# Happy-ZZX/PL-VIWO

Measured on AMD Instinct MI355X. Metric: frames/sec (track+EKF update), 752x480 mono, 250 pts+80 lines; ATE vs CPU ref, higher is better.
Workload: dtype f64

## Files before the change

### pl-viwo_amd/csrc/dense_kernels.hip

```cpp
#include "mfma_tile.hpp"
#include "update_kernels.hpp"
#include "wave_ops.hpp"

namespace plv {


static inline int cdiv(int a, int b) { return (a + b - 1) / b; }

__global__ void __launch_bounds__(256) gram_direct_kernel(const double *__restrict__ A, int lda, int nc, const int *__restrict__ acc_rows, int F,
                                                          int mp_max, double *__restrict__ G, const int *__restrict__ skip,
                                                          double *__restrict__ Gs, double *__restrict__ gv) {
  if (skip && *skip == 0) return;
  __shared__ double part[3][256];
  const int nt = (nc + 15) >> 4;
  int rem = blockIdx.x, ti = 0;
  while (rem >= nt - ti) {
    rem -= nt - ti;
    ++ti;
  }
  const int tj = ti + rem;
  const int wave = threadIdx.x >> 6, lane = threadIdx.x & 63, li = lane & 15;
  const double *ai = A + (size_t)min(ti * 16 + li, nc - 1) * lda;
  const double *aj = A + (size_t)min(tj * 16 + li, nc - 1) * lda;
  d4 acc = {0, 0, 0, 0};
  int turn = 0;
  for (int f0 = 0; f0 < F; f0 += 64) {
    const int fr = f0 + lane < F ? acc_rows[f0 + lane] : 0;
    unsigned long long mask = __ballot(fr > 0);
    while (mask) {
      const int b = __ffsll((long long)mask) - 1;
      mask &= mask - 1;
      if ((turn++ & 3) != wave) continue;
      const int rows = min(__shfl(fr, b, 64), mp_max);
      const double *af = ai + (size_t)(f0 + b) * mp_max, *bf = aj + (size_t)(f0 + b) * mp_max;
      auto fa = [&](int, int kk) { return af[kk]; };
      auto fb = [&](int kk, int) { return bf[kk]; };
      acc = mfma_tile_f64_pipe<8>(fa, fb, rows, acc);
    }
  }
  if (wave > 0) {
#pragma unroll
    for (int q = 0; q < 4; ++q) part[wave - 1][q * 64 + lane] = acc[q];
  }
  __syncthreads();
  if (wave == 0) {
#pragma unroll
    for (int q = 0; q < 4; ++q) {
      const double v = ((acc[q] + part[0][q * 64 + lane]) + part[1][q * 64 + lane]) + part[2][q * 64 + lane];
      const int i = ti * 16 + (lane >> 4) + 4 * q, j = tj * 16 + li;
      if (Gs) {
        const int k = nc - 1;
        if (i < k && j < k) Gs[(size_t)j * k + i] = v, Gs[(size_t)i * k + j] = v;
        if (i < k && j == k) gv[i] = v;
      } else if (i < nc && j < nc) {
        G[(size_t)j * nc + i] = v;
      }
    }
  }
}

__global__ void __launch_bounds__(256) ekf_dc_kernel(const double *__restrict__ W, int ldw, int r, int n,
                                                     double *__restrict__ dC, int ldc, double *__restrict__ dx,
                                                     const double *__restrict__ P, int ldp, int *__restrict__ flag, const int *__restrict__ skip,
                                                     const double *__restrict__ dW, const double *__restrict__ C1,
                                                     const double *__restrict__ d0, const int *__restrict__ use_m) {
  if (skip && *skip == 0) return;
  const bool fm = use_m && (use_m[0] | use_m[1]) != 0;
  if (fm) dW = C1;
  const int tn = (n + 1 + 15) >> 4;
  const int ntri = tn * (tn + 1) / 2;
  const int wid = blockIdx.x * 4 + (threadIdx.x >> 6);
  const int lane = threadIdx.x & 63;
  if (wid >= ntri) return;
  int ti = 0, rem = wid;
  while (rem >= tn - ti) {
    rem -= tn - ti;
    ++ti;
  }
  const int tj = ti + rem;
  const double *Wi = W + (size_t)min(ti * 16 + (lane & 15), n) * ldw;
  const double *Wj = W + (size_t)min(tj * 16 + (lane & 15), n) * ldw;
  d4 acc = {0, 0, 0, 0};
  auto fa = [&](int, int kk) { return Wi[kk]; };
  auto fb = [&](int kk, int) { return Wj[kk]; };
  acc = mfma_tile_f64_pipe<16>(fa, fb, r, acc);
#pragma unroll
  for (int q = 0; q < 4; ++q) {
    const int i = ti * 16 + (lane >> 4) + 4 * q, j = tj * 16 + (lane & 15);
    const double v = (dW && i < n && j < n) ? dW[(size_t)j * ldc + i] - acc[q] : acc[q];
    if (i < n && j < n) dC[(size_t)j * ldc + i] = v;
    if (dx && i < n && j == n) dx[i] = fm ? d0[i] - acc[q] : acc[q];
    if (P && i == j && i < n && P[(size_t)i * ldp + i] - v < 0.0) atomicOr(flag, 1);
  }
}

__global__ void __launch_bounds__(256) ekf_commit_kernel(double *__restrict__ P, int ldp, int n,
                                                         const double *__restrict__ dC, int ldc, int *__restrict__ flag,
                                                         const unsigned *__restrict__ mirror_src, unsigned *__restrict__ mirror_dst,
                                                         int mirror_words, const int *__restrict__ skip, double *__restrict__ dx,
                                                         const unsigned *__restrict__ mirror2_src, unsigned *__restrict__ mirror2_dst,
                                                         int mirror2_words,
                                                         int *__restrict__ applied_out, const int *__restrict__ cap_words, int cap,
                                                         double *__restrict__ save, unsigned *__restrict__ save_word, unsigned save_seq) {
  const bool skipped = skip && *skip == 0;
  const bool capped = cap_words && cap_words[0] != 0 && cap_words[1] >= cap;
  if (capped && blockIdx.x == 0) {
    if (threadIdx.x == 0) atomicOr(flag, 16);
    __syncthreads();
  }
  if (applied_out && blockIdx.x == 0 && threadIdx.x == 0) *applied_out = (skipped || capped || *flag != 0) ? 0 : 1;
  if (save_word && blockIdx.x == 0 && threadIdx.x == 0) *save_word = (skipped || capped || *flag != 0) ? 0u : save_seq;
  if (blockIdx.x == 0) {
    if (skipped && dx) {
      for (int i = threadIdx.x; i < n; i += blockDim.x) dx[i] = 0.0;
      __syncthreads();
    }
    if (mirror_dst)
      for (int i = threadIdx.x; i < mirror_words; i += blockDim.x) mirror_dst[i] = mirror_src[i];
  }
  if (mirror2_dst && blockIdx.x == gridDim.x - 1)
    for (int i = threadIdx.x; i < mirror2_words; i += blockDim.x) mirror2_dst[i] = mirror2_src[i];
  if (!(skipped || capped || *flag != 0)) {
    for (int idx = blockIdx.x * blockDim.x + threadIdx.x; idx < n * n; idx += gridDim.x * blockDim.x) {
      int j = idx / n, i = idx - j * n;
      if (i <= j) {
        const double u = P[(size_t)j * ldp + i];
        if (save) save[(size_t)j * n + i] = u, save[(size_t)i * n + j] = P[(size_t)i * ldp + j];
        double v = u - dC[(size_t)j * ldc + i];
        P[(size_t)j * ldp + i] = v;
        P[(size_t)i * ldp + j] = v;
      }
    }
  }
}

bool ekf_fast_fits(int r) { return r <= 192; }
static int launch_ekf_commit(plv_ctx *ctx, double *d_P, int n, int ldp, const double *dC, double *d_dx, int *d_flag, const void *mirror_src,
                             void *mirror_dst, size_t mirror_bytes);

int launch_ekf_fast(plv_ctx *ctx, double *d_P, int n, int ldp, const double *d_H, int r, int k, int ldh, const int *d_cols,
                    const double *d_res, const double *d_Rdiag, double *d_dx, int *d_flag, bool gathered, const void *mirror_src,
                    void *mirror_dst, size_t mirror_bytes) {
  int rc;
  const int ldm = r, ldw = r;
  if ((rc = ctx->d_Mt.reserve((size_t)r * (n + 1 + k) * 8)) || (rc = ctx->d_S.reserve((size_t)r * r * 8 * 2)) ||
      (rc = ctx->d_W.reserve((size_t)r * (n + 1) * 8)) || (rc = ctx->d_y.reserve((size_t)n * n * 8)))
    return rc;
  double *Mt = ctx->d_Mt.as<double>(), *S = ctx->d_S.as<double>(), *W = ctx->d_W.as<double>(), *dC = ctx->d_y.as<double>();
  launch_ekf_ms(ctx, d_P, n, ldp, d_H, r, k, ldh, d_cols, d_Rdiag, Mt, ldm, S, gathered, d_flag);
  if ((rc = launch_bchol_ekf(ctx, S, r, r, Mt, ldm, n, d_res, W, ldw, d_flag))) return rc;
  {
    ProfScope ps(ctx->prof, "ekf_dc_kernel", ctx->stream);
    int tn = cdiv(n + 1, 16);
    int waves = tn * (tn + 1) / 2;
    hipLaunchKernelGGL(ekf_dc_kernel, dim3(cdiv(waves, 4)), dim3(256), 0, ctx->stream, W, ldw, r, n, dC, n, d_dx, d_P, ldp, d_flag, ctx->skip_word,
                       (const double *)nullptr, (const double *)nullptr, (const double *)nullptr, (const int *)nullptr);
  }
  return launch_ekf_commit(ctx, d_P, n, ldp, dC, d_dx, d_flag, mirror_src, mirror_dst, mirror_bytes);
}

static int launch_ekf_commit(plv_ctx *ctx, double *d_P, int n, int ldp, const double *dC, double *d_dx, int *d_flag, const void *mirror_src,
                             void *mirror_dst, size_t mirror_bytes) {
  {
    ProfScope ps(ctx->prof, "ekf_commit_kernel", ctx->stream);
    hipLaunchKernelGGL(ekf_commit_kernel, dim3(std::min(64, cdiv(n * n, 256))), dim3(256), 0, ctx->stream, d_P, ldp, n, dC, n,
                       d_flag, (const unsigned *)mirror_src, (unsigned *)mirror_dst, (int)(mirror_bytes / 4), ctx->skip_word, d_dx,
                       (const unsigned *)(mirror_dst ? ctx->mirror2_src : nullptr), (unsigned *)(mirror_dst ? ctx->mirror2_dst : nullptr),
                       (int)((ctx->mirror2_bytes + 3) / 4), mirror_dst ? ctx->applied_word : nullptr,
                       mirror_dst ? ctx->cap_words : nullptr, ctx->cap, ctx->cov_save, ctx->cov_save_word, ctx->cov_save_seq);
    if (mirror_dst && ctx->applied_word) ctx->applied_used = true;
    if (mirror_dst && ctx->mirror2_dst) ctx->mirror2_taken = true;
  }
  PLV_HIP_CHECK(hipGetLastError());
  return PLV_OK;
}

__global__ void __launch_bounds__(256) cov_restore_kernel(double *__restrict__ P, const double *__restrict__ save, int nn,
                                                          const unsigned *__restrict__ save_word, unsigned seq) {
  if (*save_word != seq) return;
  for (int idx = blockIdx.x * blockDim.x + threadIdx.x; idx < nn; idx += gridDim.x * blockDim.x) P[idx] = save[idx];
}
int launch_cov_restore(plv_ctx *ctx, double *d_P, int n, const double *save, const unsigned *save_word, unsigned seq) {
  hipLaunchKernelGGL(cov_restore_kernel, dim3(std::min(64, cdiv(n * n, 256))), dim3(256), 0, ctx->stream, d_P, save, n * n, save_word, seq);
  PLV_HIP_CHECK(hipGetLastError());
  return PLV_OK;
}

__global__ void __launch_bounds__(256) stack_zero_rejected_kernel(double *__restrict__ A, int lda, int nc, const int *__restrict__ acc_rows, int F, int mp_max) {
  const int f = blockIdx.x;
  if (f >= F) return;
  const int keep = max(acc_rows[f], 0);
  for (int idx = threadIdx.x; idx < nc * mp_max; idx += blockDim.x) {
    const int j = idx / mp_max, i = idx - j * mp_max;
    if (i >= keep) A[(size_t)j * lda + (size_t)f * mp_max + i] = 0.0;
  }
}
__global__ void __launch_bounds__(256) stack_compact_kernel(const double *__restrict__ A, int lda, int nc, const int *__restrict__ acc_rows, int F, int mp_max,
                                                            double *__restrict__ dst, int ldd, int *__restrict__ total_out) {
  __shared__ int s_off;
  const int f = blockIdx.x;
  if (total_out && f == 0 && threadIdx.x < 64) {
    int tot = 0;
    for (int g = threadIdx.x; g < F; g += 64) tot += max(acc_rows[g], 0);
#pragma unroll
    for (int o = 32; o >= 1; o >>= 1) tot += __shfl_xor(tot, o);
    if (threadIdx.x == 0) *total_out = tot;
  }
  const int rows = max(acc_rows[f], 0);
  if (rows == 0) return;
  if (threadIdx.x < 64) {
    int part = 0;
    for (int g = threadIdx.x; g < f; g += 64) part += max(acc_rows[g], 0);
#pragma unroll
    for (int o = 32; o >= 1; o >>= 1) part += __shfl_xor(part, o);
    if (threadIdx.x == 0) s_off = part;
  }
  __syncthreads();
  const int off = s_off;
  if (off + rows > ldd) return;
  for (int idx = threadIdx.x; idx < nc * rows; idx += blockDim.x) {
    const int j = idx / rows, i = idx - j * rows;
    dst[(size_t)j * ldd + off + i] = A[(size_t)j * lda + (size_t)f * mp_max + i];
  }
}
int launch_stack_compact(plv_ctx *ctx, const double *d_A, int lda, int nc, const int *d_acc_rows, int F, int mp_max, double *d_dst, int ldd, bool exact_rows,
                         int *d_total_out) {
  if (!exact_rows) PLV_HIP_CHECK(hipMemsetAsync(d_dst, 0, (size_t)ldd * nc * 8, ctx->stream));
  ProfScope ps(ctx->prof, "stack_compact_kernel", ctx->stream);
  hipLaunchKernelGGL(stack_compact_kernel, dim3(F), dim3(256), 0, ctx->stream, d_A, lda, nc, d_acc_rows, F, mp_max, d_dst, ldd, d_total_out);
  PLV_HIP_CHECK(hipGetLastError());
  return PLV_OK;
}

int launch_stack_zero_rejected(plv_ctx *ctx, double *d_A, int lda, int nc, const int *d_acc_rows, int F, int mp_max) {
  ProfScope ps(ctx->prof, "stack_zero_rejected_kernel", ctx->stream);
  hipLaunchKernelGGL(stack_zero_rejected_kernel, dim3(F), dim3(256), 0, ctx->stream, d_A, lda, nc, d_acc_rows, F, mp_max);
  PLV_HIP_CHECK(hipGetLastError());
  return PLV_OK;
}

__global__ void __launch_bounds__(64) prior_exact_cols_kernel(const double *__restrict__ Lt, int ldl, int k, const int *__restrict__ cols,
                                                              double *__restrict__ W0, int ldw, int *__restrict__ n_near) {
  const int j = blockIdx.x;
  double *dst = W0 + (size_t)cols[j] * ldw;
  const double *src = Lt + (size_t)j * ldl;
  for (int c = threadIdx.x; c < k; c += 64) dst[c] = c <= j ? src[c] : 0.0;
  if (j == 0 && threadIdx.x == 0) {
    n_near[4] = n_near[0];
    n_near[0] = 0;
  }
}

int launch_prior_factor(plv_ctx *ctx, hipStream_t st, const double *d_P, int n, int ldp, const int *d_cols, int k) {
  int rc;
  if ((rc = ctx->d_Lt.reserve((size_t)k * k * 8)) || (rc = ctx->d_W0.reserve((size_t)k * (n + 1) * 8)) ||
      (rc = ctx->d_dW.reserve((size_t)n * n * 8)) || (rc = ctx->d_prior_near.reserve(64)))
    return rc;
  if ((rc = launch_bchol_prior(ctx, st, d_P, ldp, n, d_cols, k, ctx->d_Lt.as<double>(), k, ctx->d_W0.as<double>(), k, ctx->d_prior_near.as<int>()))) return rc;
  {
    ProfScope ps(ctx->prof, "prior_exact_cols_kernel", st);
    hipLaunchKernelGGL(prior_exact_cols_kernel, dim3(k), dim3(64), 0, st, ctx->d_Lt.as<double>(), k, k, d_cols, ctx->d_W0.as<double>(), k,
                       ctx->d_prior_near.as<int>());
  }
  {
    ProfScope ps(ctx->prof, "prior_gain_kernel", st);
    const int tn = cdiv(n + 1, 16), waves = tn * (tn + 1) / 2;
    hipLaunchKernelGGL(ekf_dc_kernel, dim3(cdiv(waves, 4)), dim3(256), 0, st, ctx->d_W0.as<double>(), k, k, n, ctx->d_dW.as<double>(), n,
                       (double *)nullptr, (const double *)nullptr, 0, (int *)nullptr, (const int *)nullptr, (const double *)nullptr,
                       (const double *)nullptr, (const double *)nullptr, (const int *)nullptr);
  }
  PLV_HIP_CHECK(hipGetLastError());
  return PLV_OK;
}

int launch_gram_information(plv_ctx *ctx, const double *d_A, int lda, int nc, const int *d_acc_rows, int F, int mp_max) {
  const int k = nc - 1, nt = cdiv(nc, 16), ntri = nt * (nt + 1) / 2;
  int rc;
  if ((rc = ctx->d_Gs.reserve(((size_t)k * k + k) * 8))) return rc;
  ProfScope ps(ctx->prof, "gram_direct_kernel", ctx->stream);
  hipLaunchKernelGGL(gram_direct_kernel, dim3(ntri), dim3(256), 0, ctx->stream, d_A, lda, nc, d_acc_rows, F, mp_max, (double *)nullptr,
                     ctx->skip_word, ctx->d_Gs.as<double>(), ctx->d_Gs.as<double>() + (size_t)k * k);
  PLV_HIP_CHECK(hipGetLastError());
  return PLV_OK;
}

int launch_ekf_whitened(plv_ctx *ctx, double *d_P, int n, int ldp, int k, const int *d_cols, double *d_dx, int *d_flag, const void *mirror_src,
                        void *mirror_dst, size_t mirror_bytes) {
  int rc;
  if ((rc = ctx->d_Mt.reserve((size_t)k * 8)) || (rc = ctx->d_S.reserve((size_t)k * k * 8)) || (rc = ctx->d_W.reserve((size_t)k * (n + 1) * 8)) ||
      (rc = ctx->d_y.reserve((size_t)n * n * 8)))
    return rc;
  double *cv = ctx->d_Mt.as<double>(), *B = ctx->d_S.as<double>(), *V = ctx->d_W.as<double>(), *dC = ctx->d_y.as<double>();
  const double *Gs = ctx->d_Gs.as<double>(), *gv = Gs + (size_t)k * k;
  if ((rc = ctx->d_C1.reserve(((size_t)n * n + n) * 8)) || (rc = ctx->d_Y0.reserve((size_t)k * (n + 1) * 8)) || (rc = ctx->d_GP.reserve((size_t)k * n * 8)))
    return rc;
  double *Y0 = ctx->d_Y0.as<double>(), *C1 = ctx->d_C1.as<double>(), *d0 = C1 + (size_t)n * n, *GP = ctx->d_GP.as<double>();
  const int *use_m = ctx->d_prior_near.as<int>();
  if (plv::knob(plv::PLV_KNOB_FORCE_FACTOR_FORM)) {
    static const int one[2] = {1, 0};
    PLV_HIP_CHECK(hipMemcpyAsync(ctx->d_prior_near.p, one, 8, hipMemcpyHostToDevice, ctx->stream));
  }
  launch_whiten_b(ctx, ctx->d_Lt.as<double>(), k, Gs, gv, cv, B, d_flag, d_P, ldp, n, d_cols, Y0, GP, d0, use_m);
// ... 13 lines not shown
```

### pl-viwo_amd/csrc/gate_core.hpp

```cpp
#pragma once
#include "blocked_chol.hpp"
#include "gate_stage.hpp"
#include "mfma_tile.hpp"
#include "wave_ops.hpp"

#ifndef GATE_STAMP
#define GATE_STAMP(id)
#endif

namespace plv {

struct GateLds {
  double S[GATE_MMAX * (GATE_MMAX + 1)];
  BcLdsT<2> bc;
  double ybuf[64];
  double passflag;
};

__device__ __forceinline__ double gate_wave_sum(double v) {
#pragma unroll
  for (int off = 32; off > 0; off >>= 1) v += __shfl_xor(v, off, 64);
  return v;
}

struct GateOps {
  static constexpr bool kStoreL = false;
  const double *S;
  const double *r;
  int rstr, mp;
  double *y;
  __device__ __forceinline__ double sym_raw(int i, int c) const {
    const int hi = min(max(i, c), mp - 1), lo = min(min(i, c), mp - 1);
    return S[lo * (GATE_MMAX + 1) + hi];
  }
  __device__ __forceinline__ double border_raw(int, int c) const { return r[(size_t)min(c, mp - 1) * rstr]; }
  __device__ __forceinline__ void scales_ready() const {}
  __device__ __forceinline__ double sym_fix(int i, int c, double g) const { return (i >= mp || c >= mp) ? (i == c ? 1.0 : 0.0) : g; }
  __device__ __forceinline__ double border_fix(int b, int c, double g) const { return (b == 0 && c < mp) ? g : 0.0; }
  __device__ __forceinline__ void store_sym(int, int, double) const {}
  __device__ __forceinline__ void store_border(int b, int c, double v) const {
    if (b == 0 && c < mp) y[c] = v;
  }
};

__host__ __device__ inline int gate_ps_doubles(int k) { return k * (k + 1) / 2 + (k + 1) / 2 + 2; }
__device__ __forceinline__ int gate_tri(int a, int b) {
  const int hi = max(a, b), lo = min(a, b);
  return hi * (hi + 1) / 2 + lo;
}
__device__ __forceinline__ void gate_stage_prior(const GateStage &g, double *Ps, const int *cols_g, int k, int tid, int nthreads) {
  int *cols_l = reinterpret_cast<int *>(Ps + k * (k + 1) / 2);
  for (int i = tid; i < k; i += nthreads) cols_l[i] = cols_g[i];
  const int w = tid >> 6, nw = nthreads >> 6, lane = tid & 63;
  for (int h0 = w; h0 < k; h0 += 8 * nw) {
    double v[8][2];
#pragma unroll
    for (int u = 0; u < 8; ++u) {
      const int hi = min(h0 + u * nw, k - 1);
      const double *row = g.P + (size_t)cols_g[hi] * g.ldp;
#pragma unroll
      for (int c = 0; c < 2; ++c) v[u][c] = row[cols_g[min(lane + 64 * c, hi)]];
    }
#pragma unroll
    for (int u = 0; u < 8; ++u) {
      const int hi = h0 + u * nw;
#pragma unroll
      for (int c = 0; c < 2; ++c) {
        const int lo = lane + 64 * c;
        if (hi < k && lo <= hi) Ps[hi * (hi + 1) / 2 + lo] = v[u][c];
      }
    }
  }
}

__device__ __forceinline__ void gate_tail(const GateStage &g, GateLds &L, const double *Ps, double *T, int f, const double *X, int ncol, int fdim,
                                          int shift, int rows, int k, const int *cols_g) {
  const int wave = threadIdx.x >> 6, lane = threadIdx.x & 63, li = lane & 15, lq = lane >> 4;
  const int mp = rows - fdim;
  const bool valid = shift == fdim && mp >= 1 && mp <= GATE_MMAX && rows >= g.min_rows;
  if (f == 0 && threadIdx.x == 0 && g.n_acc_next) *g.n_acc_next = 0;
  double chi = NAN, nrm2 = 0.0;
  if (valid) {
    const double *Hp = X + (size_t)shift * ncol + fdim;
    if (threadIdx.x == 0) {
      L.bc.bad = 0;
      L.bc.step_flag = 0;
      L.bc.rs_flag = 0;
      L.bc.n_amb = 0;
    }
    const int mt = (mp + 15) >> 4, kt = (k + 15) >> 4;
    const int ngroups = (k + 15) >> 4;
    for (int tj = wave; tj < kt; tj += 4) {
      const int jb = min(tj * 16 + li, k - 1);
      double bv[GATE_KMAX / 4];
#pragma unroll
      for (int u = 0; u < GATE_KMAX / 4; ++u) {
        const int kk = 4 * u + lq;
        const double x = Ps[kk < k ? gate_tri(kk, jb) : 0];
        bv[u] = kk < k ? x : 0.0;
      }
      for (int ti = 0; ti < mt; ++ti) {
        const double *Hr = Hp + (size_t)min(ti * 16 + li, mp - 1) * ncol + lq;
        d4 acc = {0, 0, 0, 0};
#pragma unroll
        for (int gq = 0; gq < GATE_KMAX / 16; ++gq)
          if (gq < ngroups) {
            double av[4];
#pragma unroll
            for (int u = 0; u < 4; ++u) av[u] = (16 * gq + 4 * u + lq < k) ? Hr[16 * gq + 4 * u] : 0.0;
#pragma unroll
            for (int u = 0; u < 4; ++u) acc = __builtin_amdgcn_mfma_f64_16x16x4f64(av[u], bv[4 * gq + u], acc, 0, 0, 0);
          }
#pragma unroll
        for (int q = 0; q < 4; ++q) {
          const int i = ti * 16 + lq + 4 * q, j = tj * 16 + li;
          if (i < mp && j < k) T[i * GATE_TLD + j] = acc[q];
        }
      }
    }
    __syncthreads();
    GATE_STAMP(6);
    for (int t = wave; t < mt * mt; t += 4) {
      const int ti = t / mt, tj = t - ti * mt;
      if (tj < ti) continue;
      const double *Tr = T + (size_t)min(ti * 16 + li, mp - 1) * GATE_TLD;
      const double *Hr = Hp + (size_t)min(tj * 16 + li, mp - 1) * ncol;
      d4 acc = {0, 0, 0, 0};
      auto fa = [&](int, int kk) { return Tr[kk]; };
      auto fb = [&](int kk, int) { return Hr[kk]; };
      acc = mfma_tile_f64_pipe<16>(fa, fb, k, acc);
#pragma unroll
      for (int q = 0; q < 4; ++q) {
        const int i = ti * 16 + lq + 4 * q, j = tj * 16 + li;
        if (i < mp && j < mp) L.S[i * (GATE_MMAX + 1) + j] = acc[q] + (i == j ? g.sigma2 : 0.0);
      }
    }
    __syncthreads();
    GATE_STAMP(7);
    if (wave == 0) {
      const double rv = lane < mp ? Hp[(size_t)lane * ncol + k] : 0.0;
      nrm2 = gate_wave_sum(rv * rv);
    }
    GateOps ops{L.S, Hp + k, ncol, mp, L.ybuf};
    blocked_chol<2>(ops, L.bc, mp, 1, 0.0, 0);
    __syncthreads();
    GATE_STAMP(8);
    if (wave == 0) {
      const double y = lane < mp ? L.ybuf[lane] : 0.0;
      chi = gate_wave_sum(y * y);
      if (L.bc.bad) chi = NAN;
    }
  }
  if (wave == 0 && lane == 0) {
    g.chi2[f] = chi;
    if (g.dec) g.dec[3 * f] = valid ? chi : NAN, g.dec[3 * f + 1] = (valid && mp < g.q95_n) ? g.chi2_mult * g.q95[mp] : NAN, g.dec[3 * f + 2] = valid ? sqrt(nrm2) : NAN;
    bool pass = valid && !isnan(chi);
    if (pass && g.res_norm_gate > 0.0) pass = sqrt(nrm2) < g.res_norm_gate;
    if (pass) pass = (mp < g.q95_n) && (chi < g.chi2_mult * g.q95[mp]);
    g.accepted[f] = pass ? 1 : 0;
    const bool overflow = shift == fdim && mp > GATE_MMAX;
    if (g.acc_rows) g.acc_rows[f] = pass ? mp : (overflow ? -1 : 0);
    if (g.h_accepted) g.h_accepted[f] = pass ? 1 : 0;
    if (g.h_acc_rows) g.h_acc_rows[f] = pass ? mp : (overflow ? -1 : 0);
    if (pass && g.n_acc) atomicAdd(g.n_acc, 1);
    L.passflag = pass ? 1.0 : 0.0;
  }
  if (g.probe_dst) {
    for (int i = threadIdx.x; i < g.probe_stride_a; i += blockDim.x) g.probe_dst[(size_t)f * g.probe_stride_a + i] = g.probe_src[(size_t)f * g.probe_stride_a + i];
    for (int i = threadIdx.x; i < g.probe_stride_b; i += blockDim.x)
      g.probe_dst[(size_t)g.probe_off_b + (size_t)f * g.probe_stride_b + i] = g.probe_src[(size_t)g.probe_off_b + (size_t)f * g.probe_stride_b + i];
  }
  if (g.stack) {
    __syncthreads();
    const bool pass = L.passflag != 0.0;
    if (!pass && g.stack_accepted_only) return;
    const double *Hp = X + (size_t)shift * ncol + fdim;
    double *dst = g.stack + (size_t)f * g.mp_max;
    const int rows_w = g.stack_accepted_only ? mp : g.mp_max;
    for (int i = threadIdx.x & 31; i < rows_w; i += 32)
      for (int j = threadIdx.x >> 5; j <= k; j += 8) {
        double v = 0.0;
        if (pass && i < mp) v = Hp[(size_t)i * ncol + j];
        dst[(size_t)j * g.lds + i] = v;
      }
  }
}

}
```

### pl-viwo_amd/csrc/jacobian_kernels.hip

```cpp
#include <hip/hip_runtime.h>
namespace plv {
#define JAC_NSTAMP 32
__device__ long long *g_jac_stamps = nullptr;
__device__ __forceinline__ void jac_stamp(int id) {
  long long *s = g_jac_stamps;
  if (s && threadIdx.x == 0) s[blockIdx.x * JAC_NSTAMP + id] = (long long)__builtin_amdgcn_s_memtime();
}
}
#define GATE_STAMP(id) jac_stamp(id)
#include "cam_models.hpp"
#include "gate_core.hpp"
#include "jacobian_kernels.hpp"
#include "nullspace_core.hpp"

namespace plv {

struct V3 {
  double v[3];
  __device__ double &operator[](int i) { return v[i]; }
  __device__ double operator[](int i) const { return v[i]; }
};
struct M3 {
  double m[9];
  __device__ double &operator()(int r, int c) { return m[3 * r + c]; }
// ... 615 lines not shown
  for (int i = 0; i < 2; ++i)
#pragma unroll
    for (int j = 0; j < 3; ++j) {
      hx[(size_t)(P.col_ext + j) * cstr + (2 * c + i) * rstr] = wz[3 * i] * sk(0, j) + wz[3 * i + 1] * sk(1, j) + wz[3 * i + 2] * sk(2, j);
      hx[(size_t)(P.col_ext + 3 + j) * cstr + (2 * c + i) * rstr] = wz[3 * i + j];
    }
}
__device__ __forceinline__ void rows_write_int(const JacParams &P, int c, const double *Wm, const double *dzeta, double *hx, int cstr, int rstr) {
  if (P.col_int < 0) return;
#pragma unroll
  for (int j = 0; j < 8; ++j) {
    hx[(size_t)(P.col_int + j) * cstr + (2 * c) * rstr] = Wm[0] * dzeta[j] + Wm[1] * dzeta[8 + j];
    hx[(size_t)(P.col_int + j) * cstr + (2 * c + 1) * rstr] = Wm[2] * dzeta[j] + Wm[3] * dzeta[8 + j];
  }
}

__device__ void jacobian_rows_core(const JacParams &P, int f, int o, int s0, double tm, int c, const Interp &jac, M3 R_GtoI, V3 p_IinG, double *hf,
                                   double *hx, double *rs, int cstr, int rstr) {
  double r2[2], dzn[4], dzeta[16], dznp[6], dpC_dI[18], Wm[4], wz[6], WI[12];
  M3 dpC_dpG;
  V3 lever;
  const V3 pf = ldV(P.p_FinG + 3 * f), pf_fej = ldV(P.p_FinG_fej + 3 * f);
  rows_est_part(P, pf, P.obs_uv + 2 * o, R_GtoI, p_IinG, r2, dzn, dzeta);
  rows_fej_part(P, pf_fej, jac.R, jac.p, dznp, dpC_dpG, dpC_dI, lever);
  rows_whiten_part(P, o, rows_at_clone(P, tm), dzn, dznp, dpC_dI, Wm, wz, WI);
  rows_write_res(c, Wm, r2, rs, rstr);
  rows_write_hf(P, pf_fej, c, wz, dpC_dpG, hf, cstr, rstr);
#pragma unroll
  for (int w = 0; w < 4; ++w) rows_write_pose(P.clone_col[s0 + w], c, WI, jac.Ho[w], jac.lam[w], hx, cstr, rstr);
  rows_write_dt(P, c, WI, jac.dtj, hx, cstr, rstr);
  rows_write_ext(P, c, wz, lever, hx, cstr, rstr);
  rows_write_int(P, c, Wm, dzeta, hx, cstr, rstr);
}

__device__ __forceinline__ void tri_wave_sync() {
  __builtin_amdgcn_fence(__ATOMIC_RELEASE, "workgroup");
  __builtin_amdgcn_wave_barrier();
  __builtin_amdgcn_fence(__ATOMIC_ACQUIRE, "workgroup");
}
#define PRE_STRIDE 127
#define LPRE_STRIDE 113
enum { LPRE_R2 = 70, LPRE_DZLI = 72, LPRE_ATC = 84, LPRE_WM = 85, LPRE_WLI = 89, LPRE_WI = 101 };
enum { PRE_R = 0, PRE_P = 9, PRE_HO = 12, PRE_LAM = 48, PRE_DTJ = 52, PRE_RE = 58, PRE_PE = 67,
       PRE_R2 = 70, PRE_DZN = 72, PRE_DZETA = 76, PRE_ATC = 92, PRE_WM = 93, PRE_WZ = 97, PRE_WI = 103, PRE_G = 115, PRE_LEVER = 124 };
__device__ __forceinline__ void pre_store_jac(double *pre, const Interp &j) {
#pragma unroll
  for (int i = 0; i < 9; ++i) pre[PRE_R + i] = j.R.m[i];
#pragma unroll
  for (int i = 0; i < 3; ++i) pre[PRE_P + i] = j.p[i];
#pragma unroll
  for (int w = 0; w < 4; ++w) {
#pragma unroll
    for (int i = 0; i < 9; ++i) pre[PRE_HO + 9 * w + i] = j.Ho[w].m[i];
    pre[PRE_LAM + w] = j.lam[w];
  }
#pragma unroll
  for (int i = 0; i < 6; ++i) pre[PRE_DTJ + i] = j.dtj[i];
}
__device__ __forceinline__ void pre_load_jac(const double *pre, Interp &j) {
#pragma unroll
  for (int i = 0; i < 9; ++i) j.R.m[i] = pre[PRE_R + i];
#pragma unroll
  for (int i = 0; i < 3; ++i) j.p[i] = pre[PRE_P + i];
#pragma unroll
  for (int w = 0; w < 4; ++w) {
#pragma unroll
    for (int i = 0; i < 9; ++i) j.Ho[w].m[i] = pre[PRE_HO + 9 * w + i];
    j.lam[w] = pre[PRE_LAM + w];
  }
#pragma unroll
  for (int i = 0; i < 6; ++i) j.dtj[i] = pre[PRE_DTJ + i];
}
__device__ __forceinline__ int assign_row_slots(const JacParams &P, int o0, int o1, int ld, const double *tm_l , int *s0_l, int *slot_l) {
  const int lane = threadIdx.x & 63;
  int base = 0;
  for (int ob = o0; ob < o1; ob += 64) {
    const int o = ob + lane;
    const bool have = o < o1;
    const double tm = (have ? tm_l[o - o0] : 0.0) + P.cam_dt;
    const int s0 = have ? bounding_start(P, tm) : -1;
    const unsigned long long vmask = __ballot(s0 >= 0);
    const int c = base + __popcll(vmask & ((1ull << lane) - 1ull));
    base += __popcll(vmask);
    if (have) {
      s0_l[o - o0] = s0;
      slot_l[o - o0] = (s0 >= 0 && 2 * c + 2 <= ld) ? c : -1;
    }
  }
  return base;
}
__device__ __forceinline__ void est_pose_tab(const JacParams &P, const WinTab &T, int o, int s0, double tm, M3 &R_GtoI, V3 &p_IinG) {
  if (P.res_R) {
    R_GtoI = ldM(P.res_R + 9 * o);
    p_IinG = ldV(P.res_p + 3 * o);
  } else {
    Interp est;
    interpolate_tab(P, T, s0, tm, false, est);
    R_GtoI = est.R;
    p_IinG = est.p;
  }
}

__device__ __forceinline__ void jacobian_rows_split(const JacParams &P, const V3 &pf, const V3 &pf_fej, int o0, int n_o, const int *s0_l,
                                                    const int *slot_l, const double *tm_l, const float *uv_l, double *pre, double *X, int ncol, int k) {
  const int wave = threadIdx.x >> 6, lane = threadIdx.x & 63;
  double *hf = X, *hx = X + 3, *rs = X + 3 + k;
  for (int ib = 0; ib < n_o; ib += 64) {
    const int i = ib + lane;
    const int c = i < n_o ? slot_l[i] : -1;
    const int o = o0 + i;
    double *pr = pre + (size_t)max(c, 0) * PRE_STRIDE;
    double dznp[6], dpC_dI[18];
    if (c >= 0) {
      if (wave == 0) {
        M3 dpC_dpG;
        V3 lever;
        rows_fej_part(P, pf_fej, ldM(pr + PRE_R), ldV(pr + PRE_P), dznp, dpC_dpG, dpC_dI, lever);
#pragma unroll
        for (int q = 0; q < 9; ++q) pr[PRE_G + q] = dpC_dpG.m[q];
#pragma unroll
        for (int q = 0; q < 3; ++q) pr[PRE_LEVER + q] = lever[q];
      } else if (wave == 1 && P.cam_model == PLV_CAM_EQUIDISTANT) {
        rows_est_part(P, pf, uv_l + 2 * i, ldM(pr + PRE_RE), ldV(pr + PRE_PE), pr + PRE_R2, pr + PRE_DZN, pr + PRE_DZETA);
      } else if (wave == 1) {
        double r2[2], dzn[4], dzeta[16];
        rows_est_part(P, pf, uv_l + 2 * i, ldM(pr + PRE_RE), ldV(pr + PRE_PE), r2, dzn, dzeta);
        pr[PRE_R2] = r2[0], pr[PRE_R2 + 1] = r2[1];
#pragma unroll
        for (int q = 0; q < 4; ++q) pr[PRE_DZN + q] = dzn[q];
#pragma unroll
        for (int q = 0; q < 16; ++q) pr[PRE_DZETA + q] = dzeta[q];
      } else if (wave == 2) {
        pr[PRE_ATC] = rows_at_clone(P, tm_l[i] + P.cam_dt) ? 1.0 : 0.0;
      }
    }
    __syncthreads();
    if (c >= 0 && wave == 0) {
      double dzn[4], Wm[4], wz[6], WI[12];
#pragma unroll
      for (int q = 0; q < 4; ++q) dzn[q] = pr[PRE_DZN + q];
      rows_whiten_part(P, o, pr[PRE_ATC] != 0.0, dzn, dznp, dpC_dI, Wm, wz, WI);
#pragma unroll
      for (int q = 0; q < 4; ++q) pr[PRE_WM + q] = Wm[q];
#pragma unroll
      for (int q = 0; q < 6; ++q) pr[PRE_WZ + q] = wz[q];
#pragma unroll
      for (int q = 0; q < 12; ++q) pr[PRE_WI + q] = WI[q];
    }
    __syncthreads();
    if (c >= 0) {
      double WI[12];
#pragma unroll
      for (int q = 0; q < 12; ++q) WI[q] = pr[PRE_WI + q];
      rows_write_pose(P.clone_col[s0_l[i] + wave], c, WI, ldM(pr + PRE_HO + 9 * wave), pr[PRE_LAM + wave], hx, 1, ncol);
      if (wave == 0) {
        double Wm[4], r2[2] = {pr[PRE_R2], pr[PRE_R2 + 1]}, dtj[6];
#pragma unroll
        for (int q = 0; q < 4; ++q) Wm[q] = pr[PRE_WM + q];
#pragma unroll
        for (int q = 0; q < 6; ++q) dtj[q] = pr[PRE_DTJ + q];
        rows_write_res(c, Wm, r2, rs, ncol);
        rows_write_dt(P, c, WI, dtj, hx, 1, ncol);
      } else if (wave == 1) {
        double wz[6];
#pragma unroll
        for (int q = 0; q < 6; ++q) wz[q] = pr[PRE_WZ + q];
        rows_write_ext(P, c, wz, ldV(pr + PRE_LEVER), hx, 1, ncol);
      } else if (wave == 2) {
        double Wm[4], dzeta[16];
#pragma unroll
        for (int q = 0; q < 4; ++q) Wm[q] = pr[PRE_WM + q];
#pragma unroll
        for (int q = 0; q < 16; ++q) dzeta[q] = pr[PRE_DZETA + q];
        rows_write_int(P, c, Wm, dzeta, hx, 1, ncol);
      } else {
        double wz[6];
#pragma unroll
        for (int q = 0; q < 6; ++q) wz[q] = pr[PRE_WZ + q];
        rows_write_hf(P, pf_fej, c, wz, ldM(pr + PRE_G), hf, 1, ncol);
      }
    }
    __syncthreads();
  }
}

struct FusedLds {
  int ns, tab, tri, pre, cam, idx, end;
};
__host__ __device__ inline FusedLds fused_lds_layout(int ld, int ncol, int fdim, int n_tab, int max_obs, bool with_tri) {
  const bool lines = fdim == 6;
  FusedLds L;
  L.ns = ld * ncol;
  L.tab = (L.ns + nullspace_wy_scratch(ld, fdim) + 7) & ~7;
  L.tri = L.tab + n_tab * (int)(sizeof(WinTab) / 8);
  L.pre = L.tri + (with_tri && !lines ? tri_smem_doubles(max_obs) : 0);
  L.cam = L.pre + (ld / 2 < max_obs ? ld / 2 : max_obs) * (lines ? LPRE_STRIDE : PRE_STRIDE);
  L.idx = L.cam + max_obs * 12 * (lines ? 2 : 1);
  L.end = L.idx + (lines ? 5 : 3) * max_obs + (max_obs * (lines ? 13 : 9) + 7) / 8 + 1;
  return L;
}
static_assert(sizeof(WinTab) % 8 == 0, "fused_lds_layout counts WinTab in doubles");

__global__ void __launch_bounds__(256) __attribute__((amdgpu_waves_per_eu(2))) jacobian_nullspace_kernel(JacParams P, int F, GatherArgs g, PointTriStage tri, GateStage gate) {
  extern __shared__ double jsm[];
  __shared__ int s_rows, s_base;
  __shared__ double tri_tot[32], s_tri[5];
  __shared__ double s_ct[JAC_MAX_WIN / 2 + 3];
  __shared__ int s_ccol[JAC_MAX_WIN / 2 + 3];
  if ((int)blockIdx.x >= F) {
    gather_cov_block(g, blockIdx.x - F);
    return;
  }
  int f = blockIdx.x;
  if (P.spec_order) {
    if ((int)blockIdx.x >= *P.spec_count) return;
    f = P.spec_order[blockIdx.x];
  }
  const int wave = threadIdx.x >> 6, lane = threadIdx.x & 63;
  double touch = 0.0;
  for (int off = threadIdx.x * 128; off < P.in_bytes; off += 256 * 128) touch += *(const volatile double *)(P.in_base + off);
  const int ld = P.ld, k = P.k, ncol = 3 + k + 1, max_obs = tri.max_obs;
  const FusedLds lay = fused_lds_layout(ld, ncol, 3, 2 * max(P.n_clones - 3, 0), max_obs, tri.on != 0);
  double *X = jsm, *piv = jsm + lay.ns, *tri_smem = jsm + lay.tri, *pre = jsm + lay.pre, *cam = jsm + lay.cam;
  WinTab *tab = reinterpret_cast<WinTab *>(jsm + lay.tab);
  double *tm_l = jsm + lay.idx;
  float *uv_l = reinterpret_cast<float *>(tm_l + max_obs), *uvn_l = uv_l + 2 * max_obs;
  int *s0_l = reinterpret_cast<int *>(uvn_l + 2 * max_obs), *slot_l = s0_l + max_obs;
  unsigned char *valid_l = reinterpret_cast<unsigned char *>(slot_l + max_obs);
  jac_stamp(0);
  const int o0 = P.obs_ptr[f], o1 = P.obs_end ? P.obs_end[f] : P.obs_ptr[f + 1];
  if ((int)threadIdx.x < P.n_clones) s_ct[threadIdx.x] = P.clone_time[threadIdx.x], s_ccol[threadIdx.x] = P.clone_col[threadIdx.x];
  for (int i = threadIdx.x; i < o1 - o0; i += blockDim.x) {
    tm_l[i] = P.obs_time[o0 + i];
    uv_l[2 * i] = P.obs_uv[2 * (o0 + i)], uv_l[2 * i + 1] = P.obs_uv[2 * (o0 + i) + 1];
    if (tri.on) uvn_l[2 * i] = tri.uvn[2 * (o0 + i)], uvn_l[2 * i + 1] = tri.uvn[2 * (o0 + i) + 1];
  }
  for (int i = threadIdx.x; i < ld * ncol; i += blockDim.x) X[i] = 0.0;
  if (f == 0 && P.cols_out)
    for (int i = threadIdx.x; i < k; i += blockDim.x) P.cols_out[i] = P.cols_in[i];
  __syncthreads();
  P.clone_time = s_ct, P.clone_col = s_ccol;
  if (wave == 0) {
    const int base = assign_row_slots(P, o0, o1, ld, tm_l, s0_l, slot_l);
    if (lane == 0) s_base = base;
    jac_stamp(15);
  }
  build_window_tables(P, tab);
  jac_stamp(2);
  if (wave == 0) {
    for (int i = lane; i < o1 - o0; i += 64) {
      const int s0 = s0_l[i], c = slot_l[i];
      valid_l[i] = s0 >= 0;
      if (s0 < 0) continue;
      M3 R_GtoI;
      V3 p_IinG;
      est_pose_tab(P, tab[2 * s0], o0 + i, s0, tm_l[i] + P.cam_dt, R_GtoI, p_IinG);
      if (c >= 0) {
        double *pr = pre + (size_t)c * PRE_STRIDE;
#pragma unroll
        for (int q = 0; q < 9; ++q) pr[PRE_RE + q] = R_GtoI.m[q];
#pragma unroll
        for (int q = 0; q < 3; ++q) pr[PRE_PE + q] = p_IinG[q];
      }
      if (tri.on) {
        const M3 R_GtoC = mm(ldM(P.R_ItoC), R_GtoI);
        const V3 p_CinG = vsub(p_IinG, mv(tp(R_GtoC), ldV(P.p_IinC)));
#pragma unroll
        for (int q = 0; q < 9; ++q) cam[12 * i + q] = R_GtoC.m[q];
#pragma unroll
        for (int q = 0; q < 3; ++q) cam[12 * i + 9 + q] = p_CinG[q];
      }
    }
    if (tri.on) {
      tri_wave_sync();
      triangulate_feature(P, f, 0, o1 - o0, cam, valid_l, uvn_l, uv_l, tri.opt, tri.p_out, tri.ok_out, tri.err_out, max_obs, tri_smem, tri_tot, true, s_tri);
    }
  } else {
    for (int i = threadIdx.x - 64; i < o1 - o0; i += 192) {
      const int c = slot_l[i];
      if (c < 0) continue;
      Interp jac;
      const int s0 = s0_l[i];
      interpolate_tab(P, tab[2 * s0 + 1], s0, tm_l[i] + P.cam_dt, true, jac);
      pre_store_jac(pre + (size_t)c * PRE_STRIDE, jac);
    }
    if (gate.on) gate_stage_prior(gate, reinterpret_cast<double *>(reinterpret_cast<char *>(jsm) + gate.ps_off), P.cols_in, k, threadIdx.x - 64, 192);
  }
  __threadfence_block();
  __syncthreads();
  jac_stamp(1);
  bool selected;
  V3 pf, pf_fej;
  if (tri.on) {
    selected = P.sel_flags[f] && s_tri[3] != 0.0 && s_tri[4] < 3.0;
    pf = pf_fej = ldV(s_tri);
  } else {
    selected = !P.tri_ok || candidate_selected(P, f);
    pf = ldV(P.p_FinG + 3 * f), pf_fej = ldV(P.p_FinG_fej + 3 * f);
  }
  if (selected) {
    jacobian_rows_split(P, pf, pf_fej, o0, o1 - o0, s0_l, slot_l, tm_l, uv_l, pre, X, ncol, k);
    if (threadIdx.x == 0) {
      s_rows = min(2 * s_base, ld & ~1);
      P.rows[f] = 2 * s_base;
      if (P.spec_pass) atomicAdd(P.spec_pass, 1);
    }
  } else if (threadIdx.x == 0) {
    s_rows = 0;
    P.rows[f] = 0;
  }
  __syncthreads();
  jac_stamp(3);
  const int rows = s_rows;
  GateLds &gl = *reinterpret_cast<GateLds *>(reinterpret_cast<char *>(jsm) + gate.lds_off);
  const double *gPs = reinterpret_cast<const double *>(reinterpret_cast<char *>(jsm) + gate.ps_off);
  double *gT = reinterpret_cast<double *>(reinterpret_cast<char *>(jsm) + gate.t_off);
  if ((tri.on || P.tri_ok) && rows == 0) {
    if (gate.on) gate_tail(gate, gl, gPs, gT, f, X, ncol, 3, 0, 0, k, P.cols_in);
    return;
  }
  const int shift = rows > 3 ? 3 : 0;
  if (shift) nullspace_householder_wy<3>(X, piv, rows, ncol);
  jac_stamp(4);
  double *hf = P.Hf + (size_t)f * 3 * ld, *hx = P.Hx + (size_t)f * k * ld, *rs = P.res + (size_t)f * ld;
  for (int j = gate.on ? ncol : (int)threadIdx.x; j < ncol; j += blockDim.x) {
    double *dst = j < 3 ? hf + j * ld : (j < 3 + k ? hx + (size_t)(j - 3) * ld : rs);
    const int off = j < 3 ? 0 : shift;
    for (int i0 = 0; i0 < ld; i0 += 8) {
      double v[8];
#pragma unroll
      for (int u = 0; u < 8; ++u) {
        const int r = i0 + u + off;
        v[u] = r < ld ? X[r * ncol + j] : 0.0;
      }
#pragma unroll
      for (int u = 0; u < 8; ++u)
        if (i0 + u < ld) dst[i0 + u] = v[u];
    }
  }
  jac_stamp(5);
  if (gate.on) gate_tail(gate, gl, gPs, gT, f, X, ncol, 3, shift, min(rows, ld), k, P.cols_in);
  if (touch == 1.2345678e300) P.rows[f] = -1;
  jac_stamp(9);
}

__device__ __forceinline__ void campose_one(const JacParams &P, int o, double *__restrict__ poses , unsigned char *__restrict__ valid,
                            double *__restrict__ imu) {
  const double tm = P.obs_time[o] + P.cam_dt;
  const int s0 = bounding_start(P, tm);
  valid[o] = s0 >= 0;
  if (s0 < 0) return;
  M3 R_GtoI;
  V3 p_IinG;
  if (P.res_R) {
    R_GtoI = ldM(P.res_R + 9 * o);
    p_IinG = ldV(P.res_p + 3 * o);
  } else {
    Interp est;
    interpolate(P, s0, tm, false, false, est);
    R_GtoI = est.R;
    p_IinG = est.p;
  }
  if (imu) {
#pragma unroll
    for (int i = 0; i < 9; ++i) imu[12 * o + i] = R_GtoI.m[i];
#pragma unroll
    for (int i = 0; i < 3; ++i) imu[12 * o + 9 + i] = p_IinG[i];
  }
  const M3 R_GtoC = mm(ldM(P.R_ItoC), R_GtoI);
  const V3 p_CinG = vsub(p_IinG, mv(tp(R_GtoC), ldV(P.p_IinC)));
#pragma unroll
  for (int i = 0; i < 9; ++i) poses[12 * o + i] = R_GtoC.m[i];
#pragma unroll
  for (int i = 0; i < 3; ++i) poses[12 * o + 9 + i] = p_CinG[i];
}

__device__ int cpi_find(const double *t, int n, double x) {
  int lo = 0, hi = n;
  while (lo < hi) {
    const int mid = (lo + hi) >> 1;
    if (t[mid] < x) lo = mid + 1; else hi = mid;
  }
  return (lo < n && t[lo] == x) ? lo : -1;
}
__device__ int clone_find(const CpiParams &C, double x) {
  for (int i = 0; i < C.n_clones; ++i)
    if (C.clone_time[i] == x) return i;
  return -1;
}
__global__ void __launch_bounds__(64) cpi_pose_kernel(CpiParams C, const double *__restrict__ tq, double *__restrict__ Rout,
                                                      double *__restrict__ pout, unsigned char *__restrict__ ok) {
  const int q = blockIdx.x * blockDim.x + threadIdx.x;
  if (q >= C.n_q) return;
  ok[q] = 0;
  const double t = tq[q];
  const int n = C.n;
  M3 R_I0toIk;
  V3 alpha;
  double clone_t, dt;
  const int e = cpi_find(C.t, n, t);
  if (e >= 0 && clone_find(C, C.clone_t[e]) >= 0) {
    R_I0toIk = ldM(C.R + 9 * e);
    alpha = ldV(C.alpha + 3 * e);
    clone_t = C.clone_t[e];
    dt = C.dt[e];
  } else {
    if (n == 0 || t < C.t[0] || t > C.t[n - 1]) return;
    int lo = 0, hi = n;
    while (lo < hi) {
      const int mid = (lo + hi) >> 1;
      if (C.t[mid] < t) lo = mid + 1; else hi = mid;
    }
    const int i0 = (t == C.t[0]) ? 0 : lo - 1;
    int up = lo;
    while (up < n && C.t[up] <= t) ++up;
    const int i1 = (t == C.t[n - 1]) ? n - 1 : up;
    if (C.clone_t[i0] != C.clone_t[i1]) return;
    if (C.clone_t[i0] < C.clone_time[0]) return;
    const double lambda = (t - C.t[i0]) / (C.t[i1] - C.t[i0]);
    const M3 R0 = ldM(C.R + 9 * i0), R1 = ldM(C.R + 9 * i1);
    R_I0toIk = mm(exp_so3(vsc(log_so3(mm(R1, tp(R0))), lambda)), R0);
    const V3 a0 = ldV(C.alpha + 3 * i0), a1 = ldV(C.alpha + 3 * i1);
    alpha = vadd(vsc(a0, 1 - lambda), vsc(a1, lambda));
    clone_t = C.clone_t[i0];
    dt = t - clone_t;
  }
  const int ci = clone_find(C, clone_t), vi = cpi_find(C.t, n, clone_t);
  if (ci < 0 || vi < 0) return;
  const M3 RGtoI0 = ldM(C.clone_R + 9 * ci);
  const V3 p0 = ldV(C.clone_p + 3 * ci), v0 = ldV(C.v + 3 * vi);
  const V3 g{{C.gravity[0], C.gravity[1], C.gravity[2]}};
  const M3 RGtoI = mm(R_I0toIk, RGtoI0);
  V3 p = vadd(p0, vsc(v0, dt));
  p = vsub(p, vsc(vsc(vsc(g, 0.5), dt), dt));
  p = vadd(p, mv(tp(RGtoI0), alpha));
#pragma unroll
  for (int i = 0; i < 9; ++i) Rout[9 * q + i] = RGtoI.m[i];
#pragma unroll
  for (int i = 0; i < 3; ++i) pout[3 * q + i] = p[i];
// ... 412 lines not shown
#pragma unroll
    for (int j = 0; j < 3; ++j) {
      double so = 0, sp = 0;
#pragma unroll
      for (int q = 0; q < 3; ++q) {
        so += a[6 * i + q] * A00(q, j);
        sp += a[6 * i + q] * A03(q, j);
      }
#pragma unroll
      for (int q = 0; q < 3; ++q) {
        so += a[6 * i + 3 + q] * A30(q, j);
        sp += a[6 * i + 3 + q] * 0.0;
      }
      x[6 * i + j] = so;
      x[6 * i + 3 + j] = sp;
    }
}
__device__ __forceinline__ void line_whiten_part(const JacParams &P, int o, bool at_clone, const double *dzli, const M3 &A00, const M3 &A30, const M3 &A03,
                                                 double *Wm, double *wli, double *WI) {
  double HI[12];
  line_times_dli(dzli, A00, A30, A03, HI);
  double Rn[4] = {P.sigma_pix * P.sigma_pix, 0, 0, P.sigma_pix * P.sigma_pix};
  if (!at_clone && P.use_pol_cov) {
#pragma unroll
    for (int i = 0; i < 2; ++i)
#pragma unroll
      for (int j = 0; j < 2; ++j) {
        double s = 0;
#pragma unroll
        for (int q = 0; q < 6; ++q) s += HI[6 * i + q] * (q < 3 ? P.intr_ori_cov : P.intr_pos_cov) * HI[6 * j + q];
        Rn[2 * i + j] += s;
      }
  } else if (!at_clone && P.use_imu_cov) {
    add_imu_cov(P, o, HI, Rn);
  }
  const double l00 = sqrt(Rn[0]), l10 = Rn[2] / l00, l11 = sqrt(Rn[3] - l10 * l10);
  const double m00 = sqrt(l00), m10 = l10 / m00, m11 = sqrt(l11 - m10 * m10);
#pragma unroll
  for (int col = 0; col < 2; ++col) {
    const double b0 = col == 0 ? 1.0 : 0.0, b1 = col == 1 ? 1.0 : 0.0;
    const double y0 = b0 / m00, y1 = (b1 - m10 * y0) / m11;
    const double x1 = y1 / m11, x0 = (y0 - m10 * x1) / m00;
    Wm[col] = x0;
    Wm[2 + col] = x1;
  }
#pragma unroll
  for (int j = 0; j < 6; ++j) {
    wli[j] = Wm[0] * dzli[j] + Wm[1] * dzli[6 + j];
    wli[6 + j] = Wm[2] * dzli[j] + Wm[3] * dzli[6 + j];
  }
  line_times_dli(wli, A00, A30, A03, WI);
}
__device__ __forceinline__ void line_write_hf(int c, const double *wli, const M3 &Re, const M3 &Rsk, double *hf, int cstr, int rstr) {
#pragma unroll
  for (int i = 0; i < 2; ++i)
#pragma unroll
    for (int j = 0; j < 3; ++j) {
      double a = 0, b = 0;
#pragma unroll
      for (int q = 0; q < 3; ++q) {
        a += wli[6 * i + q] * Re(q, j);
        b += wli[6 * i + q] * Rsk(q, j);
      }
#pragma unroll
      for (int q = 0; q < 3; ++q) {
        a += wli[6 * i + 3 + q] * 0.0;
        b += wli[6 * i + 3 + q] * Re(q, j);
      }
      hf[(size_t)j * cstr + (2 * c + i) * rstr] = a;
      hf[(size_t)(3 + j) * cstr + (2 * c + i) * rstr] = b;
    }
}

__device__ void line_rows(const JacParams &P, int l, int o, int s0, double tm, int c, double *hf, double *hx, double *rs, int cstr,
                          int rstr, const WinTab *tab = nullptr) {
  const V3 nG = ldV(P.line_FinG + 6 * l), vG = ldV(P.line_FinG + 6 * l + 3);
  Interp jac;
  if (tab)
    interpolate_tab(P, tab[2 * s0 + 1], s0, tm, true, jac);
  else
    interpolate(P, s0, tm, true, true, jac);
  M3 Re;
  V3 pe;
  if (P.res_R) {
    Re = ldM(P.res_R + 9 * o);
    pe = ldV(P.res_p + 3 * o);
  } else {
    Interp est;
    if (tab)
      interpolate_tab(P, tab[2 * s0], s0, tm, false, est);
    else
      interpolate(P, s0, tm, false, false, est);
    Re = est.R;
    pe = est.p;
  }
  double r2[2], dzli[12], Wm[4], wli[12], WI[12];
  M3 Rsk, A00, A30, A03;
  line_est_part(P, nG, vG, P.seg_uv + 4 * o, Re, pe, r2, dzli, Rsk);
  line_fej_part(nG, vG, jac.R, jac.p, A00, A30, A03);
  line_whiten_part(P, o, rows_at_clone(P, tm), dzli, A00, A30, A03, Wm, wli, WI);
  rows_write_res(c, Wm, r2, rs, rstr);
  line_write_hf(c, wli, Re, Rsk, hf, cstr, rstr);
#pragma unroll
  for (int w = 0; w < 4; ++w) rows_write_pose(P.clone_col[s0 + w], c, WI, jac.Ho[w], jac.lam[w], hx, cstr, rstr);
  rows_write_dt(P, c, WI, jac.dtj, hx, cstr, rstr);
}

__global__ void __launch_bounds__(64) line_jacobian_kernel(JacParams P) {
  const int l = blockIdx.x;
  const int ld = P.ld, k = P.k;
  double *hf = P.Hf + (size_t)l * 6 * ld, *hx = P.Hx + (size_t)l * k * ld, *rs = P.res + (size_t)l * ld;
  for (int i = threadIdx.x; i < 6 * ld; i += 64) hf[i] = 0.0;
  for (int i = threadIdx.x; i < k * ld; i += 64) hx[i] = 0.0;
  for (int i = threadIdx.x; i < ld; i += 64) rs[i] = 0.0;
  __syncthreads();
  if (P.tri_ok && !candidate_selected(P, l)) {
    if (threadIdx.x == 0) P.rows[l] = 0;
    return;
  }
  const int o0 = P.obs_ptr[l], o1 = P.obs_ptr[l + 1];
  int base = 0;
  for (int ob = o0; ob < o1; ob += 64) {
    const int o = ob + threadIdx.x;
    const bool have = o < o1;
    const double tm = (have ? P.obs_time[o] : 0.0) + P.cam_dt;
    const int s0 = have ? bounding_start(P, tm) : -1;
    const unsigned long long vmask = __ballot(s0 >= 0);
    const int c = base + __popcll(vmask & ((1ull << threadIdx.x) - 1ull));
    base += __popcll(vmask);
    if (s0 >= 0 && 2 * c + 2 <= ld) line_rows(P, l, o, s0, tm, c, hf, hx, rs, ld, 1);
  }
  if (threadIdx.x == 0) P.rows[l] = 2 * base;
}

__device__ void line_triangulate_one(const JacParams &P, int l, int o0, int o1, const double *cam, const double *imu, const unsigned char *valid,
                                     const float *seg_uvn, const double *anchor, bool has_anchor, double *out, unsigned char &ok);
struct LineTriStage {
  int on, max_obs;
  double *cam, *imu;
  unsigned char *valid;
  double *out_g;
  unsigned char *ok_g;
};
__device__ __forceinline__ void line_rows_split(const JacParams &P, const V3 &nG, const V3 &vG, int o0, int n_o, const int *s0_l, const int *slot_l,
                                                const double *tm_l, const float *seg_l, double *pre, double *X, int ncol, int k) {
  const int wave = threadIdx.x >> 6, lane = threadIdx.x & 63;
  double *hf = X, *hx = X + 6, *rs = X + 6 + k;
  for (int ib = 0; ib < n_o; ib += 64) {
    const int i = ib + lane;
    const int c = i < n_o ? slot_l[i] : -1;
    const int o = o0 + i;
    double *pr = pre + (size_t)max(c, 0) * LPRE_STRIDE;
    M3 A00, A30, A03;
    M3 Re, Rsk;
    if (c >= 0) {
      if (wave == 0) {
        line_fej_part(nG, vG, ldM(pr + PRE_R), ldV(pr + PRE_P), A00, A30, A03);
      } else if (wave == 1) {
        double r2[2], dzli[12];
        Re = ldM(pr + PRE_RE);
        line_est_part(P, nG, vG, seg_l + 4 * i, Re, ldV(pr + PRE_PE), r2, dzli, Rsk);
        pr[LPRE_R2] = r2[0], pr[LPRE_R2 + 1] = r2[1];
#pragma unroll
        for (int q = 0; q < 12; ++q) pr[LPRE_DZLI + q] = dzli[q];
      } else if (wave == 2) {
        pr[LPRE_ATC] = rows_at_clone(P, tm_l[i] + P.cam_dt) ? 1.0 : 0.0;
      }
    }
    __syncthreads();
    if (c >= 0 && wave == 0) {
      double dzli[12], Wm[4], wli[12], WI[12];
#pragma unroll
      for (int q = 0; q < 12; ++q) dzli[q] = pr[LPRE_DZLI + q];
      line_whiten_part(P, o, pr[LPRE_ATC] != 0.0, dzli, A00, A30, A03, Wm, wli, WI);
#pragma unroll
      for (int q = 0; q < 4; ++q) pr[LPRE_WM + q] = Wm[q];
#pragma unroll
      for (int q = 0; q < 12; ++q) pr[LPRE_WLI + q] = wli[q], pr[LPRE_WI + q] = WI[q];
    }
    __syncthreads();
    if (c >= 0) {
      double WI[12];
#pragma unroll
      for (int q = 0; q < 12; ++q) WI[q] = pr[LPRE_WI + q];
      rows_write_pose(P.clone_col[s0_l[i] + wave], c, WI, ldM(pr + PRE_HO + 9 * wave), pr[PRE_LAM + wave], hx, 1, ncol);
      if (wave == 0) {
        double Wm[4], r2[2] = {pr[LPRE_R2], pr[LPRE_R2 + 1]}, dtj[6];
#pragma unroll
        for (int q = 0; q < 4; ++q) Wm[q] = pr[LPRE_WM + q];
#pragma unroll
        for (int q = 0; q < 6; ++q) dtj[q] = pr[PRE_DTJ + q];
        rows_write_res(c, Wm, r2, rs, ncol);
        rows_write_dt(P, c, WI, dtj, hx, 1, ncol);
      } else if (wave == 1) {
        double wli[12];
#pragma unroll
        for (int q = 0; q < 12; ++q) wli[q] = pr[LPRE_WLI + q];
        line_write_hf(c, wli, Re, Rsk, hf, 1, ncol);
      }
    }
    __syncthreads();
  }
}

__device__ __forceinline__ void jpl_left_update_dev(const double *Qin, const double *d, double *M) {
  double a[3] = {0.5 * d[0], 0.5 * d[1], 0.5 * d[2]}, b = 1.0;
  const double nd = sqrt(a[0] * a[0] + a[1] * a[1] + a[2] * a[2] + 1.0);
  a[0] /= nd, a[1] /= nd, a[2] /= nd, b /= nd;
  const double v[3] = {Qin[0], Qin[1], Qin[2]}, w0 = Qin[3];
  double r[4];
  r[0] = b * v[0] - (a[1] * v[2] - a[2] * v[1]) + a[0] * w0;
  r[1] = b * v[1] - (a[2] * v[0] - a[0] * v[2]) + a[1] * w0;
  r[2] = b * v[2] - (a[0] * v[1] - a[1] * v[0]) + a[2] * w0;
  r[3] = -(a[0] * v[0] + a[1] * v[1] + a[2] * v[2]) + b * w0;
  if (r[3] < 0) {
#pragma unroll
    for (int i = 0; i < 4; ++i) r[i] = -r[i];
  }
  const double nr = sqrt(r[0] * r[0] + r[1] * r[1] + r[2] * r[2] + r[3] * r[3]);
  double Q[4];
#pragma unroll
  for (int i = 0; i < 4; ++i) Q[i] = r[i] / nr;
  const double x = Q[0], y = Q[1], z = Q[2], w = Q[3], c = 2 * w * w - 1;
  M[0] = c + 2 * x * x, M[1] = 2 * w * z + 2 * x * y, M[2] = -2 * w * y + 2 * x * z;
  M[3] = -2 * w * z + 2 * y * x, M[4] = c + 2 * y * y, M[5] = 2 * w * x + 2 * y * z;
  M[6] = 2 * w * y + 2 * z * x, M[7] = -2 * w * x + 2 * z * y, M[8] = c + 2 * z * z;
}

__global__ void __launch_bounds__(256) line_jacobian_nullspace_kernel(JacParams P, int L, GatherArgs g, JacParams Pt, LineTriStage tri, GateStage gate) {
  extern __shared__ double jsm[];
  __shared__ int s_rows, s_base, s_ok;
  __shared__ double s_line[6];
  __shared__ double s_ct[JAC_MAX_WIN / 2 + 3];
  __shared__ int s_ccol[JAC_MAX_WIN / 2 + 3];
  __shared__ double s_cR[(JAC_MAX_WIN / 2 + 3) * 9], s_cp[(JAC_MAX_WIN / 2 + 3) * 3], s_cal[9 + 3 + 8 + 1], s_anchor[3];
  __shared__ unsigned char s_has;
  if (P.chain_dx && *P.chain_status != 0) return;
  if ((int)blockIdx.x >= L) {
    gather_cov_block(g, blockIdx.x - L);
    return;
  }
  const int l = blockIdx.x, wave = threadIdx.x >> 6, lane = threadIdx.x & 63;
  double touch = 0.0;
  for (int off = threadIdx.x * 128; off < P.in_bytes; off += 256 * 128) touch += *(const volatile double *)(P.in_base + off);
  const int ld = P.ld, k = P.k, ncol = 6 + k + 1, max_obs = tri.max_obs, nwin = max(P.n_clones - 3, 0);
  const FusedLds lay = fused_lds_layout(ld, ncol, 6, (tri.on ? 3 : 2) * nwin, max_obs, tri.on != 0);
  double *X = jsm, *piv = jsm + lay.ns, *pre = jsm + lay.pre, *cam = jsm + lay.cam, *imu = cam + (size_t)max_obs * 12;
  WinTab *tab = reinterpret_cast<WinTab *>(jsm + lay.tab);
  double *tm_l = jsm + lay.idx;
  float *uv_l = reinterpret_cast<float *>(tm_l + max_obs), *uvn_l = uv_l + 4 * max_obs;
  int *s0_l = reinterpret_cast<int *>(uvn_l + 4 * max_obs), *slot_l = s0_l + max_obs, *s0t_l = slot_l + max_obs;
  unsigned char *valid_l = reinterpret_cast<unsigned char *>(s0t_l + max_obs);
  jac_stamp(0);
  const int o0 = P.obs_ptr[l], o1 = P.obs_ptr[l + 1];
  if ((int)threadIdx.x < P.n_clones) s_ct[threadIdx.x] = P.clone_time[threadIdx.x], s_ccol[threadIdx.x] = P.clone_col[threadIdx.x];
  for (int i = threadIdx.x; i < o1 - o0; i += blockDim.x) {
    tm_l[i] = P.obs_time[o0 + i];
#pragma unroll
    for (int q = 0; q < 4; ++q) uv_l[4 * i + q] = P.seg_uv[4 * (o0 + i) + q];
    if (tri.on)
#pragma unroll
      for (int q = 0; q < 4; ++q) uvn_l[4 * i + q] = Pt.seg_uvn[4 * (o0 + i) + q];
  }
  for (int i = threadIdx.x; i < ld * ncol; i += blockDim.x) X[i] = 0.0;
  if (l == 0 && P.cols_out)
    for (int i = threadIdx.x; i < k; i += blockDim.x) P.cols_out[i] = P.cols_in[i];
  __syncthreads();
  P.clone_time = s_ct, P.clone_col = s_ccol, Pt.clone_time = s_ct;
  if (P.chain_dx && *P.chain_applied != 0) {
    const double *dx = P.chain_dx;
    const int N = P.n_clones, t = threadIdx.x;
    if (t < N) {
      const int id = P.chain_id[t];
#pragma unroll
      for (int q = 0; q < 3; ++q) s_cp[3 * t + q] = id >= 0 ? P.clone_p[3 * t + q] + dx[id + 3 + q] : P.clone_p[3 * t + q];
      if (id >= 0) {
        jpl_left_update_dev(P.chain_q + 4 * t, dx + id, s_cR + 9 * t);
      } else {
#pragma unroll
        for (int q = 0; q < 9; ++q) s_cR[9 * t + q] = P.clone_R[9 * t + q];
      }
    } else if (t == 64) {
      const int id = P.chain_id[N];
      if (id >= 0) {
        jpl_left_update_dev(P.chain_qe, dx + id, s_cal);
#pragma unroll
        for (int q = 0; q < 3; ++q) s_cal[9 + q] = P.p_IinC[q] + dx[id + 3 + q];
      } else {
#pragma unroll
        for (int q = 0; q < 9; ++q) s_cal[q] = P.R_ItoC[q];
#pragma unroll
        for (int q = 0; q < 3; ++q) s_cal[9 + q] = P.p_IinC[q];
      }
    } else if (t == 65) {
      const int id = P.chain_id[N + 1];
#pragma unroll
      for (int q = 0; q < 8; ++q) s_cal[12 + q] = id >= 0 ? P.K[q] + dx[id + q] : P.K[q];
    } else if (t == 66) {
      const int id = P.chain_id[N + 2];
      s_cal[20] = id >= 0 ? P.cam_dt + dx[id] : P.cam_dt;
    }
    __syncthreads();
    P.clone_R = s_cR, P.clone_p = s_cp;
#pragma unroll
    for (int q = 0; q < 9; ++q) P.R_ItoC[q] = s_cal[q];
#pragma unroll
    for (int q = 0; q < 3; ++q) P.p_IinC[q] = s_cal[9 + q];
#pragma unroll
    for (int q = 0; q < 8; ++q) P.K[q] = s_cal[12 + q];
    P.cam_dt = s_cal[20];
  }
  if (wave == 0) {
    const int base = assign_row_slots(P, o0, o1, ld, tm_l, s0_l, slot_l);
    if (lane == 0) s_base = base;
    jac_stamp(15);
  } else if (wave == 1 && tri.on) {
    for (int i = lane; i < o1 - o0; i += 64) s0t_l[i] = bounding_start(Pt, tm_l[i] + Pt.cam_dt);
  }
  build_window_tables(P, tab, tri.on ? Pt.clone_R : nullptr, tri.on ? Pt.clone_p : nullptr);
  jac_stamp(2);
  if (wave == 0) {
    if (tri.on) {
      for (int i = lane; i < o1 - o0; i += 64) {
        const int s0 = s0t_l[i];
        valid_l[i] = s0 >= 0;
        if (s0 < 0) continue;
        M3 R_GtoI;
        V3 p_IinG;
        est_pose_tab(Pt, tab[2 * nwin + s0], o0 + i, s0, tm_l[i] + Pt.cam_dt, R_GtoI, p_IinG);
#pragma unroll
        for (int q = 0; q < 9; ++q) imu[12 * i + q] = R_GtoI.m[q];
#pragma unroll
        for (int q = 0; q < 3; ++q) imu[12 * i + 9 + q] = p_IinG[q];
        const M3 R_GtoC = mm(ldM(Pt.R_ItoC), R_GtoI);
        const V3 p_CinG = vsub(p_IinG, mv(tp(R_GtoC), ldV(Pt.p_IinC)));
#pragma unroll
        for (int q = 0; q < 9; ++q) cam[12 * i + q] = R_GtoC.m[q];
#pragma unroll
        for (int q = 0; q < 3; ++q) cam[12 * i + 9 + q] = p_CinG[q];
      }
      if (Pt.anc_ptr && lane == 0) {
        unsigned char has = 0;
        for (int c = Pt.anc_ptr[l]; c < Pt.anc_ptr[l + 1] && !has; ++c) {
          const int pf = Pt.anc_f[c];
          if (pf >= 0 && Pt.anc_tri_ok[pf]) {
            s_anchor[0] = Pt.anc_tri_p[3 * pf], s_anchor[1] = Pt.anc_tri_p[3 * pf + 1], s_anchor[2] = Pt.anc_tri_p[3 * pf + 2];
            has = 1;
          } else if (Pt.anc_has_old[c]) {
            s_anchor[0] = Pt.anc_old[3 * c], s_anchor[1] = Pt.anc_old[3 * c + 1], s_anchor[2] = Pt.anc_old[3 * c + 2];
            has = 1;
          }
        }
        s_has = has;
      }
      tri_wave_sync();
      jac_stamp(10);
      double out_l[6] = {0, 0, 0, 0, 0, 0};
      unsigned char ok_l = 0;
      const bool has_anchor = Pt.anc_ptr ? s_has != 0 : (Pt.has_pt && Pt.has_pt[l]);
      line_triangulate_one(Pt, l, 0, o1 - o0, cam, imu, valid_l, uvn_l, Pt.anc_ptr ? s_anchor : Pt.anchor_pt + 3 * l, has_anchor, out_l, ok_l);
      if (lane == 0) {
#pragma unroll
        for (int i = 0; i < 6; ++i) tri.out_g[6 * l + i] = out_l[i], s_line[i] = out_l[i];
        tri.ok_g[l] = ok_l;
        s_ok = ok_l;
      }
    }
  } else {
    for (int i = threadIdx.x - 64; i < o1 - o0; i += 192) {
      const int c = slot_l[i];
      if (c < 0) continue;
      const int s0 = s0_l[i];
      double *pr = pre + (size_t)c * LPRE_STRIDE;
      Interp jac;
      interpolate_tab(P, tab[2 * s0 + 1], s0, tm_l[i] + P.cam_dt, true, jac);
      pre_store_jac(pr, jac);
      M3 Re;
      V3 pe;
      est_pose_tab(P, tab[2 * s0], o0 + i, s0, tm_l[i] + P.cam_dt, Re, pe);
#pragma unroll
      for (int q = 0; q < 9; ++q) pr[PRE_RE + q] = Re.m[q];
#pragma unroll
      for (int q = 0; q < 3; ++q) pr[PRE_PE + q] = pe[q];
    }
    if (gate.on) gate_stage_prior(gate, reinterpret_cast<double *>(reinterpret_cast<char *>(jsm) + gate.ps_off), P.cols_in, k, threadIdx.x - 64, 192);
  }
  __threadfence_block();
  __syncthreads();
  jac_stamp(1);
  bool selected;
  V3 nG, vG;
  if (tri.on) {
    selected = P.sel_flags[l] && s_ok;
    nG = ldV(s_line), vG = ldV(s_line + 3);
  } else {
    selected = !P.tri_ok || candidate_selected(P, l);
    nG = ldV(P.line_FinG + 6 * l), vG = ldV(P.line_FinG + 6 * l + 3);
  }
  if (selected) {
    line_rows_split(P, nG, vG, o0, o1 - o0, s0_l, slot_l, tm_l, uv_l, pre, X, ncol, k);
    if (threadIdx.x == 0) {
      s_rows = min(2 * s_base, ld & ~1);
      P.rows[l] = 2 * s_base;
    }
  } else if (threadIdx.x == 0) {
    s_rows = 0;
    P.rows[l] = 0;
  }
  __syncthreads();
  jac_stamp(3);
  const int rows = s_rows;
  GateLds &gl = *reinterpret_cast<GateLds *>(reinterpret_cast<char *>(jsm) + gate.lds_off);
  const double *gPs = reinterpret_cast<const double *>(reinterpret_cast<char *>(jsm) + gate.ps_off);
  double *gT = reinterpret_cast<double *>(reinterpret_cast<char *>(jsm) + gate.t_off);
  if ((tri.on || P.tri_ok) && rows == 0) {
    if (gate.on) gate_tail(gate, gl, gPs, gT, l, X, ncol, 6, 0, 0, k, P.cols_in);
    return;
  }
  const int shift = rows > 6 ? 6 : 0;
  if (shift) nullspace_householder_wy<6>(X, piv, rows, ncol);
  jac_stamp(4);
  double *hf = P.Hf + (size_t)l * 6 * ld, *hx = P.Hx + (size_t)l * k * ld, *rs = P.res + (size_t)l * ld;
  for (int j = gate.on ? ncol : (int)threadIdx.x; j < ncol; j += blockDim.x) {
    double *dst = j < 6 ? hf + j * ld : (j < 6 + k ? hx + (size_t)(j - 6) * ld : rs);
    const int off = j < 6 ? 0 : shift;
    for (int i0 = 0; i0 < ld; i0 += 8) {
      double v[8];
#pragma unroll
      for (int u = 0; u < 8; ++u) {
        const int r = i0 + u + off;
        v[u] = r < ld ? X[r * ncol + j] : 0.0;
      }
#pragma unroll
      for (int u = 0; u < 8; ++u)
        if (i0 + u < ld) dst[i0 + u] = v[u];
    }
  }
  jac_stamp(5);
  if (gate.on) gate_tail(gate, gl, gPs, gT, l, X, ncol, 6, shift, min(rows, ld), k, P.cols_in);
  if (touch == 1.2345678e300) P.rows[l] = -1;
  jac_stamp(9);
}

__device__ void line_triangulate_one(const JacParams &P, int l, int o0, int o1, const double *cam, const double *imu, const unsigned char *valid,
                                     const float *seg_uvn, const double *anchor, bool has_anchor, double *out, unsigned char &ok);
__global__ void __launch_bounds__(64) line_triangulate_kernel(JacParams P, double *cam, double *imu, unsigned char *valid, double *out_g,
                                                              unsigned char *ok_g) {
  const int l = blockIdx.x;
  const int o0 = P.obs_ptr[l], o1 = P.obs_ptr[l + 1];
  for (int o = o0 + (int)threadIdx.x; o < o1; o += 64) campose_one(P, o, cam, valid, imu);
  __threadfence_block();
  __syncthreads();
  double out_l[6] = {0, 0, 0, 0, 0, 0};
  unsigned char ok_l = 0;
  line_triangulate_one(P, l, o0, o1, cam, imu, valid, P.seg_uvn, P.anchor_pt + 3 * l, P.has_pt && P.has_pt[l], out_l, ok_l);
  if (threadIdx.x == 0) {
#pragma unroll
    for (int i = 0; i < 6; ++i) out_g[6 * l + i] = out_l[i];
    ok_g[l] = ok_l;
  }
}
__device__ void line_triangulate_one(const JacParams &P, int l, int o0, int o1, const double *cam, const double *imu, const unsigned char *valid,
                                     const float *seg_uvn, const double *anchor, bool has_anchor, double *out , unsigned char &ok) {
  int first = -1, nvalid = 0;
  for (int o = o0; o < o1; ++o)
    if (valid[o]) {
      if (first < 0) first = o;
      ++nvalid;
    }
  if (nvalid < 2) return;
  const int D = P.lineD ? P.lineD[l] : 0;
  if (D > 0 && has_anchor) {
    const M3 R = ldM(imu + 12 * first);
    const V3 e{{D == 1 ? 1.0 : 0.0, D == 2 ? 1.0 : 0.0, D == 3 ? 1.0 : 0.0}};
    const V3 dir = mv(tp(R), e);
    const V3 mom = cross3(ldV(anchor), dir);
#pragma unroll
    for (int i = 0; i < 3; ++i) {
      out[i] = mom[i];
      out[3 + i] = dir[i];
    }
    ok = 1;
    return;
  }
  const M3 R0 = ldM(cam + 12 * first);
  const V3 p0 = ldV(cam + 12 * first + 9);
  const float *u0 = seg_uvn + 4 * first;
  const V3 p11{{(double)u0[0], (double)u0[1], 1.0}}, p12{{(double)u0[2], (double)u0[3], 1.0}};
  const V3 n0 = cross3(p11, p12);
  const double pl0[4] = {n0[0], n0[1], n0[2], 0.0};
  V3 dsum{{0, 0, 0}}, nsum{{0, 0, 0}};
  double dnorm = 0;
  int cnt = 0;
  for (int o = first + 1; o < o1; ++o) {
    if (!valid[o]) continue;
    const M3 Ri = ldM(cam + 12 * o);
    const V3 pi = ldV(cam + 12 * o + 9);
    const M3 R0i = mm(Ri, tp(R0));
    const V3 pi0 = mv(R0, vsub(pi, p0));
    const float *um = seg_uvn + 4 * o;
    V3 p31{{(double)um[0], (double)um[1], 1.0}}, p32{{(double)um[2], (double)um[3], 1.0}};
    p31 = vadd(mv(tp(R0i), p31), pi0);
    p32 = vadd(mv(tp(R0i), p32), pi0);
    const V3 nn = cross3(vsub(p31, pi0), vsub(p32, pi0));
    const double pl1[4] = {nn[0], nn[1], nn[2], -dot3(pi0, cross3(p31, p32))};
    V3 n1{{pl0[0], pl0[1], pl0[2]}}, n2{{pl1[0], pl1[1], pl1[2]}};
    n1 = vsc(n1, 1 / vnorm(n1));
    n2 = vsc(n2, 1 / vnorm(n2));
    const double cth = dot3(n1, n2) / (vnorm(n1) * vnorm(n2));
    if (fabs(cth) >= 0.99) continue;
#define PLV_DP(i, j) (pl0[i] * pl1[j] - pl1[i] * pl0[j])
    const V3 head{{PLV_DP(0, 3), PLV_DP(1, 3), PLV_DP(2, 3)}}, tail{{-PLV_DP(1, 2), PLV_DP(0, 2), -PLV_DP(0, 1)}};
#undef PLV_DP
    dsum = vadd(dsum, tail);
    nsum = vadd(nsum, head);
    dnorm += vnorm(tail);
    ++cnt;
  }
  if (cnt == 0) return;
  const V3 rhead = vsc(dsum, 1 / dnorm), rtail = vsc(nsum, 1.0 / cnt);
  const M3 R0t = tp(R0);
  const V3 vW = mv(R0t, rhead);
  const V3 nW = vadd(mv(R0t, rtail), mv(skew3(p0), mv(R0t, rhead)));
#pragma unroll
  for (int i = 0; i < 3; ++i) {
    out[i] = nW[i];
    out[3 + i] = vW[i];
  }
  ok = 1;
}

#define TRY_STAMP(x)          \
  do {                        \
    const int _rc = (x);      \
    if (_rc != PLV_OK) return _rc; \
  } while (0)
struct JacStampHost {
  bool on = plv::knob(plv::PLV_KNOB_KERNEL_STAMPS);
  long long *d = nullptr;
  int cap = 0;
  struct Acc {
    const char *name;
    double sum[JAC_NSTAMP] = {}, mx[JAC_NSTAMP] = {}, slowest = 0;
    long n[JAC_NSTAMP] = {}, launches = 0;
  } acc[2] = {{"tri_jacobian_nullspace_kernel"}, {"line_tri_jacobian_nullspace_kernel"}};
  int arm(hipStream_t s, int blocks) {
    if (blocks > cap) {
      if (d) (void)hipFree(d);
      cap = blocks + 64;
      PLV_HIP_CHECK(hipMalloc(&d, (size_t)cap * JAC_NSTAMP * 8));
      PLV_HIP_CHECK(hipMemcpyToSymbol(HIP_SYMBOL(g_jac_stamps), &d, sizeof(d)));
    }
    PLV_HIP_CHECK(hipMemsetAsync(d, 0, (size_t)blocks * JAC_NSTAMP * 8, s));
    return PLV_OK;
  }
  int collect(hipStream_t s, int blocks, int which) {
    PLV_HIP_CHECK(hipStreamSynchronize(s));
    std::vector<long long> h((size_t)blocks * JAC_NSTAMP);
    PLV_HIP_CHECK(hipMemcpy(h.data(), d, h.size() * 8, hipMemcpyDeviceToHost));
    Acc &a = acc[which];
    double slow = 0;
    for (int b = 0; b < blocks; ++b) {
      const long long *t = &h[(size_t)b * JAC_NSTAMP];
      if (!t[0] || !t[9]) continue;
      slow = std::max(slow, (double)(t[9] - t[0]));
      if (!t[4]) continue;
      for (int i = 1; i < JAC_NSTAMP; ++i)
        if (t[i]) a.sum[i] += (double)(t[i] - t[0]), a.mx[i] = std::max(a.mx[i], (double)(t[i] - t[0])), ++a.n[i];
    }
    a.slowest += slow;
    ++a.launches;
    return PLV_OK;
  }
  ~JacStampHost() {
    if (!on) return;
    static const char *label[JAC_NSTAMP] = {"start", "triangulated", "window tables", "rows built", "null space", "block written", "gate: T", "gate: S",
                                            "gate: factor", "end", "tri: camera poses", "tri: linear solve", "tri: refined", "gate: map staged", "gate: T first column", "row slots",
                                            "LM pass 1", "LM pass 2", "LM pass 3", "LM pass 4", "LM pass 5", "LM pass 6", "LM pass 7", "LM pass 8", "LM pass 9", "LM pass 10", "LM pass 11", "LM pass 12+",
                                            "", "", "", ""};
    static const int order[] = {15, 2, 10, 11, 16, 17, 18, 19, 20, 21, 22, 23, 24, 25, 26, 27, 12, 1, 3, 4, 5, 13, 14, 6, 7, 8, 9};
    for (const Acc &a : acc) {
      if (!a.launches) continue;
      fprintf(stderr, "[plv stamps] %s: %ld launches, slowest workgroup %.0f cycles on average\n", a.name, a.launches, a.slowest / (double)a.launches);
      for (int i : order)
        if (a.n[i]) fprintf(stderr, "[plv stamps]   %-20s @ %8.0f mean  %8.0f max  (%ld workgroups)\n", label[i], a.sum[i] / (double)a.n[i], a.mx[i], a.n[i]);
    }
  }
};
static JacStampHost &jac_stamps() {
  static JacStampHost h;
  return h;
}

int launch_line_jacobians(plv_ctx *ctx, const JacParams &P) {
  ProfScope ps(ctx->prof, "line_jacobian_kernel", ctx->stream);
  hipLaunchKernelGGL(line_jacobian_kernel, dim3(P.n_feat), dim3(64), 0, ctx->stream, P);
  PLV_HIP_CHECK(hipGetLastError());
  return PLV_OK;
}

int launch_line_jacobians_projected(plv_ctx *ctx, const JacParams &P, const GatherArgs *g, int gather_blocks, const JacParams *Pt, double *d_cam,
                                    double *d_imu, unsigned char *d_valid, double *d_lines, unsigned char *d_ok, int max_obs) {
  ProfScope ps(ctx->prof, Pt ? "line_tri_jacobian_nullspace_kernel" : "line_jacobian_nullspace_kernel", ctx->stream);
  if (2 * (P.n_clones - 3) > JAC_MAX_WIN) {
    set_last_error("line jacobians: %d clones exceed the window table (%d)", P.n_clones, JAC_MAX_WIN / 2 + 3);
    return PLV_E_CAPACITY;
  }
  max_obs = std::max(max_obs, 1);
  const FusedLds lay = fused_lds_layout(P.ld, 6 + P.k + 1, 6, (Pt ? 3 : 2) * std::max(P.n_clones - 3, 0), max_obs, Pt != nullptr);
  size_t shm = (size_t)lay.end * sizeof(double);
  const size_t lds_cap = 160 * 1024 - static_smem_bytes((const void *)line_jacobian_nullspace_kernel);
  if (shm > lds_cap) {
    set_last_error("line jacobians: block of %zu bytes exceeds LDS", shm);
    return PLV_E_CAPACITY;
  }
  GatherArgs none{};
  LineTriStage tri{Pt ? 1 : 0, max_obs, d_cam, d_imu, d_valid, d_lines, d_ok};
  GateStage gate = ctx->gate_stage;
  ctx->gate_stage.on = 0;
  const size_t gate_off = ((size_t)lay.tab * sizeof(double) + 63) & ~(size_t)63;
  const size_t t_off = (gate_off + sizeof(GateLds) + 63) & ~(size_t)63;
  const size_t ps_off = (std::max(shm, t_off + (size_t)GATE_MMAX * GATE_TLD * sizeof(double)) + 63) & ~(size_t)63;
  const size_t gate_end = ps_off + (size_t)gate_ps_doubles(P.k) * sizeof(double);
  if (P.k > GATE_KMAX || gate_end > lds_cap) gate.on = 0;
  if (gate.on) {
    gate.lds_off = (int)gate_off, gate.ps_off = (int)ps_off, gate.t_off = (int)t_off;
    shm = gate_end;
  }
  ctx->gate_stage_taken = gate.on != 0;
  PLV_HIP_CHECK(ensure_dyn_smem((const void *)line_jacobian_nullspace_kernel, (int)shm));
  if (jac_stamps().on) TRY_STAMP(jac_stamps().arm(ctx->stream, P.n_feat));
  hipLaunchKernelGGL(line_jacobian_nullspace_kernel, dim3(P.n_feat + (g ? gather_blocks : 0)), dim3(256), shm, ctx->stream, P, P.n_feat,
                     g ? *g : none, Pt ? *Pt : P, tri, gate);
  PLV_HIP_CHECK(hipGetLastError());
  if (jac_stamps().on) TRY_STAMP(jac_stamps().collect(ctx->stream, P.n_feat, 1));
  return PLV_OK;
}

int launch_triangulate_lines(plv_ctx *ctx, const JacParams &P, double *d_poses, double *d_imu, unsigned char *d_valid,
                             double *d_lines, unsigned char *d_ok) {
  {
    ProfScope ps(ctx->prof, "line_triangulate_kernel", ctx->stream);
    hipLaunchKernelGGL(line_triangulate_kernel, dim3(P.n_feat), dim3(64), 0, ctx->stream, P, d_poses, d_imu, d_valid, d_lines, d_ok);
  }
  PLV_HIP_CHECK(hipGetLastError());
  return PLV_OK;
}

int launch_triangulate(plv_ctx *ctx, const JacParams &P, double *d_poses, unsigned char *d_valid, const float *d_uvn,
                       const plv_tri_options &opt, double *d_p, unsigned char *d_ok, double *d_err, int max_obs) {
  {
    ProfScope ps(ctx->prof, "triangulate_kernel", ctx->stream);
    const size_t shm = (size_t)std::max(max_obs, 1) * (sizeof(TriObs) + TRI_TERMS * 8 + 4) + 16;
    if (shm > 150 * 1024) {
      set_last_error("triangulation: a track of %d observations exceeds LDS", max_obs);
      return PLV_E_CAPACITY;
    }
    PLV_HIP_CHECK(ensure_dyn_smem((const void *)triangulate_kernel, (int)shm));
    hipLaunchKernelGGL(triangulate_kernel, dim3(P.n_feat), dim3(64), shm, ctx->stream, P, d_poses, d_valid, d_uvn, opt, d_p, d_ok, d_err,
                       std::max(max_obs, 1));
  }
  PLV_HIP_CHECK(hipGetLastError());
  return PLV_OK;
}

int launch_jacobians_projected(plv_ctx *ctx, const JacParams &P, const GatherArgs *g, int gather_blocks, const plv_tri_options *tri_opt,
                               double *d_poses, unsigned char *d_valid, const float *d_uvn, double *d_p, unsigned char *d_ok, double *d_err, int max_obs) {
  ProfScope ps(ctx->prof, tri_opt ? "tri_jacobian_nullspace_kernel" : "jacobian_nullspace_kernel", ctx->stream);
  if (2 * (P.n_clones - 3) > JAC_MAX_WIN) {
    set_last_error("jacobians: %d clones exceed the window table (%d)", P.n_clones, JAC_MAX_WIN / 2 + 3);
    return PLV_E_CAPACITY;
  }
  max_obs = std::max(max_obs, 1);
  const FusedLds lay = fused_lds_layout(P.ld, 3 + P.k + 1, 3, 2 * std::max(P.n_clones - 3, 0), max_obs, tri_opt != nullptr);
  size_t shm = (size_t)lay.end * sizeof(double);
  const size_t lds_cap = 160 * 1024 - static_smem_bytes((const void *)jacobian_nullspace_kernel);
  if (shm > lds_cap) {
    set_last_error("jacobians: feature block of %zu bytes exceeds LDS", shm);
    return PLV_E_CAPACITY;
  }
  GatherArgs none{};
  PointTriStage tri{};
  tri.max_obs = max_obs;
  if (tri_opt) tri = PointTriStage{1, max_obs, d_poses, d_valid, d_uvn, *tri_opt, d_p, d_ok, d_err};
  GateStage gate = ctx->gate_stage;
  ctx->gate_stage.on = 0;
  const size_t gate_off = ((size_t)lay.tab * sizeof(double) + 63) & ~(size_t)63;
  const size_t t_off = (gate_off + sizeof(GateLds) + 63) & ~(size_t)63;
  const size_t ps_off = (std::max(shm, t_off + (size_t)GATE_MMAX * GATE_TLD * sizeof(double)) + 63) & ~(size_t)63;
  const size_t gate_end = ps_off + (size_t)gate_ps_doubles(P.k) * sizeof(double);
  if (P.k > GATE_KMAX || gate_end > lds_cap) gate.on = 0;
  if (gate.on) {
    gate.lds_off = (int)gate_off, gate.ps_off = (int)ps_off, gate.t_off = (int)t_off;
    shm = gate_end;
  }
  ctx->gate_stage_taken = gate.on != 0;
  PLV_HIP_CHECK(ensure_dyn_smem((const void *)jacobian_nullspace_kernel, (int)shm));
  if (jac_stamps().on) TRY_STAMP(jac_stamps().arm(ctx->stream, P.n_feat));
  const int wg_feat = P.spec_order ? std::max(1, std::min(P.n_feat, spec_grid(P.max_sel))) : P.n_feat;
  hipLaunchKernelGGL(jacobian_nullspace_kernel, dim3(wg_feat + (g ? gather_blocks : 0)), dim3(256), shm, ctx->stream, P, wg_feat,
                     g ? *g : none, tri, gate);
  PLV_HIP_CHECK(hipGetLastError());
  if (jac_stamps().on) TRY_STAMP(jac_stamps().collect(ctx->stream, P.n_feat, 0));
  return PLV_OK;
}

__global__ void __launch_bounds__(1024) spec_select_kernel(SpecSelectArgs A) {
  __shared__ int s_wave[16], s_base;
  const int lane = threadIdx.x & 63, wave = threadIdx.x >> 6;
  if (threadIdx.x == 0) s_base = 0;
  __syncthreads();
  for (int f0 = 0; f0 < A.F; f0 += blockDim.x) {
    const int f = f0 + threadIdx.x;
    bool in_pool = false;
    if (f < A.F) {
      const int li = A.li[f], m = A.meta[f];
      bool survived = false;
      if (li >= 0 && li < A.n_flow && A.flow_mask[li]) {
        const float x = A.flow_p1[2 * li], y = A.flow_p1[2 * li + 1];
        survived = !(x < 0 || y < 0 || (int)x >= A.W || (int)y >= A.H);
      }
      const int n_old = A.obs_ptr[f + 1] - A.obs_ptr[f] - (li >= 0 ? 1 : 0);
      const int n_use = n_old + ((survived && (m & 2)) ? 1 : 0);
      in_pool = ((m & 1) || !((m & 8) || survived)) && n_use >= 2;
    }
    const unsigned long long b = __ballot(in_pool);
    if (lane == 0) s_wave[wave] = __popcll(b);
    __syncthreads();
    int before = s_base;
    for (int w = 0; w < wave; ++w) before += s_wave[w];
    const int rank = before + __popcll(b & ((1ull << lane) - 1ull));
    if (in_pool && rank < A.grid) A.order[rank] = f;
    __syncthreads();
    if (threadIdx.x == 0) {
      int tot = 0;
      for (int w = 0; w < (int)(blockDim.x >> 6); ++w) tot += s_wave[w];
      s_base += tot;
    }
    __syncthreads();
  }
  const int count = s_base;
  const bool over = count > A.grid;
  if (threadIdx.x == 0) A.words[0] = count, A.words[1] = over ? 1 : 0, A.words[2] = over ? 0 : count, A.words[3] = (!over && count > A.max_sel) ? 1 : 0, A.words[4] = 0;
  if (threadIdx.x == 0 && A.zero_word) *A.zero_word = 0;
  if (A.cols_out)
    for (int i = threadIdx.x; i < A.k; i += blockDim.x) A.cols_out[i] = A.cols_in[i];
  for (int f = threadIdx.x; f < A.F; f += blockDim.x) {
    const int li = A.li[f], m = A.meta[f], o0 = A.obs_ptr[f], o1 = A.obs_ptr[f + 1];
    bool survived = false;
    float x = 0.f, y = 0.f;
    if (li >= 0 && li < A.n_flow && A.flow_mask[li]) {
      x = A.flow_p1[2 * li], y = A.flow_p1[2 * li + 1];
      survived = !(x < 0 || y < 0 || (int)x >= A.W || (int)y >= A.H);
    }
    const int n_old = o1 - o0 - (li >= 0 ? 1 : 0);
    const bool with_new = survived && (m & 2);
    const int n_use = n_old + (with_new ? 1 : 0);
    const bool in_pool = ((m & 1) || !((m & 8) || survived)) && n_use >= 2;
    const int n_valid = (int)A.prevalid[f] + ((with_new && (m & 4)) ? 1 : 0);
    A.member[f] = in_pool ? 1 : 0;
    A.sel_flags[f] = (in_pool && !over && n_valid >= 2) ? 1 : 0;
    A.obs_end[f] = (in_pool && !over) ? o0 + n_use : o0;
    if (in_pool && with_new) {
      const int o = o0 + n_old;
      A.obs_uv[2 * o] = x, A.obs_uv[2 * o + 1] = y;
      A.obs_uvn[2 * o] = A.flow_n1[2 * li], A.obs_uvn[2 * o + 1] = A.flow_n1[2 * li + 1];
    }
    if (!in_pool || over) {
      A.rows_out[f] = 0;
      A.tri_p[3 * f] = A.tri_p[3 * f + 1] = A.tri_p[3 * f + 2] = 0.0;
      A.tri_err[f] = 0.0;
      A.tri_ok[f] = 0;
      if (A.chi2) A.chi2[f] = NAN;
      if (A.accepted) A.accepted[f] = 0;
      if (A.acc_rows) A.acc_rows[f] = 0;
    }
  }
}
int launch_spec_select(plv_ctx *ctx, const SpecSelectArgs &A) {
  ProfScope ps(ctx->prof, "spec_select_kernel", ctx->stream);
  hipLaunchKernelGGL(spec_select_kernel, dim3(1), dim3(1024), 0, ctx->stream, A);
  PLV_HIP_CHECK(hipGetLastError());
  return PLV_OK;
}

int launch_jacobians(plv_ctx *ctx, const JacParams &P) {
  ProfScope ps(ctx->prof, "jacobian_kernel", ctx->stream);
  if (2 * (P.n_clones - 3) > JAC_MAX_WIN) {
    set_last_error("jacobians: %d clones exceed the window table (%d)", P.n_clones, JAC_MAX_WIN / 2 + 3);
    return PLV_E_CAPACITY;
  }
  hipLaunchKernelGGL(jacobian_kernel, dim3(P.n_feat), dim3(128), 0, ctx->stream, P);
  PLV_HIP_CHECK(hipGetLastError());
  return PLV_OK;
}

}
```

### pl-viwo_amd/csrc/plv_api.hip

```cpp
#include <algorithm>
#include <cstdarg>
#include <dlfcn.h>
#include <cmath>
#include <mutex>

#include "plv_ctx.hpp"
#include "update_kernels.hpp"
#include "update_state.hpp"

namespace plv {

static thread_local char g_err[512] = "";
void set_last_error(const char *fmt, ...) {
  va_list ap;
  va_start(ap, fmt);
  vsnprintf(g_err, sizeof(g_err), fmt, ap);
  va_end(ap);
}

double chi2_quantile(int dof, double p);

Roctx::Roctx() {
  if (!getenv("PLV_ROCTX")) return;
  for (const char *name : {"librocprofiler-sdk-roctx.so", "libroctx64.so"}) {
// ... 725 lines not shown
  const int F_guard = us->bF;
  us->pending_F = 0;
  ctx->probe_done = false;
  if (F_guard < 1 || ctx->cov_n < 1) {
    set_last_error("plv_msckf_update_resident: no staged batch / covariance");
    return PLV_E_BADARG;
  }
  const int F = us->bF, fdim = us->bfdim, k = us->bk, ld = us->bld, n = ctx->cov_n;
  size_t nHf = (size_t)F * fdim * ld, nHx = (size_t)F * k * ld, nr = (size_t)F * ld;
  TRY(ctx->d_chi2.reserve((size_t)F * 8));
  double *wHf;
  if (us->b_single_use) {
    wHf = us->bHf.as<double>();
    us->b_single_use = false;
    us->bF = 0;
  } else {
    TRY(us->bwork.reserve((nHf + nHx + nr) * 8));
    PLV_HIP_CHECK(plv::memcpy_async(us->bwork.p, us->bHf.p, (nHf + nHx + nr) * 8, hipMemcpyDeviceToDevice, ctx->stream));
    wHf = us->bwork.as<double>();
  }
  double *wHx = wHf + nHf, *wres = wHx + nHx;

  const int mp_max = (us->b_on_device_rows ? ld : us->bmaxrows) - fdim;
  if (mp_max < 1) {
    set_last_error("plv_msckf_update: no feature has more than fdim rows");
    return PLV_E_BADARG;
  }
  const int nc = k + 1;
  const int Mtot = F * mp_max;
  TRY(ctx->stack_of(fdim).reserve_units((size_t)F, (size_t)std::max(ctx->cfg.num_features, 64), (size_t)mp_max * nc * 8));
  size_t tmp_elems = (size_t)std::max(Mtot / (2 * nc) + 2, 16) * nc * nc;
  {
    const size_t nt = (size_t)(nc + 15) / 16, ntri = nt * (nt + 1) / 2;
    tmp_elems = std::max(tmp_elems, (size_t)((Mtot + 63) / 64) * ntri * 256 + (size_t)nc * nc);
  }
  TRY(ctx->d_stack2.reserve(tmp_elems * 8));

  double *d_dx;
  int *d_flag;
  unsigned char *d_acc;
  int *d_acc_rows;
  TRY(result_buf(ctx, us, n, F, &d_dx, &d_flag, &d_acc, &d_acc_rows, fdim));
  plv::DevBuf &resbuf = us->result_of(fdim);

  const bool projected = us->b_projected;
  const bool gathers_valid = projected && us->b_gather_token != 0 && us->b_gather_token == ctx->gather_stamp;
  us->b_gather_token = 0;
  const bool prior_was_pending = ctx->prior_pending;
  const bool prefetched = prior_was_pending && ctx->prior_k == k && gathers_valid;
  ctx->prior_pending = false;
  const size_t rb = result_rows_off(n, F) + (size_t)F * 4;
  plv::PinBuf &hpin = ctx->res_pin(fdim);
  TRY(hpin.reserve(rb));
  struct SkipGuard {
    plv_ctx *c;
    ~SkipGuard() { c->skip_word = nullptr; }
  } skip_guard{ctx};
  const bool whiten = whitened_route(us, Mtot, k);
  bool aux_open = prior_was_pending;
  auto aux_join = [&]() -> int {
    if (!aux_open) return PLV_OK;
    aux_open = false;
    PLV_HIP_CHECK(hipStreamWaitEvent(ctx->stream, ctx->aux_join, 0));
    return PLV_OK;
  };
  const bool probing = ctx->probe && !us->graph_mode;
  auto start_prior = [&]() -> int {
    TRY(aux_join());
    TRY(prior_mark(ctx, true));
    TRY(prior_start(ctx, us->bcols_of(fdim).as<int>(), k));
    aux_open = true;
    return PLV_OK;
  };
  auto enqueue = [&]() -> int {
  if (whiten && !prefetched && !probing) TRY(start_prior());
  if (!projected) {
    TRY(launch_nullspace(ctx, F, fdim, k, ld, us->brows.as<int>(), wHf, wHx, wres, ctx->d_P.as<double>(), n, n, us->bcols_of(fdim).as<int>()));
  } else if (!gathers_valid) {
    TRY(launch_gather_cov(ctx, ctx->d_P.as<double>(), n, n, us->bcols_of(fdim).as<int>(), k));
  }
  Chi2Args a{};
  a.P = ctx->d_P.as<double>();
  a.ldp = n;
  a.k = k;
  a.ld = ld;
  a.fdim_off = fdim;
  a.rows = us->brows.as<int>();
  a.Hx = wHx;
  a.res = wres;
  a.cols = us->bcols_of(fdim).as<int>();
  a.sigma2 = sigma2;
  a.chi2 = ctx->d_chi2.as<double>();
  a.dec = nullptr;
  if (ctx->decision_trace && fdim == 3) {
    TRY(ctx->d_gate_dec.reserve((size_t)F * 24));
    a.dec = ctx->d_gate_dec.as<double>();
    ctx->dec_gate = true;
  } else if (ctx->decision_trace) {
    TRY(ctx->d_gate_dec_l.reserve((size_t)F * 24));
    a.dec = ctx->d_gate_dec_l.as<double>();
    ctx->dec_F_l = F;
  }
  a.stack = ctx->stack_of(fdim).as<double>();
  a.lds = Mtot;
  a.mp_max = mp_max;
  a.chi2_mult = chi2_mult;
  a.res_norm_gate = res_norm_gate;
  a.q95 = us->q95.as<double>();
  a.q95_n = Q95_N;
  a.min_rows = fdim == 3 ? 4 : 5;
  a.accepted = d_acc;
  a.acc_rows = d_acc_rows;
  a.n_acc = d_flag + 1;
  a.stack_accepted_only = (Mtot > k && k <= 192 && whiten) ? 1 : 0;
  ctx->skip_word = (Mtot > k ? k <= 192 : ekf_fast_fits(Mtot)) ? d_flag + 1 : nullptr;
  const bool probe = ctx->probe && !us->graph_mode;
  if (probe) {
    char *hb = hpin.as<char>();
    a.h_accepted = (unsigned char *)(hb + (size_t)n * 8 + 16);
    a.h_acc_rows = (int *)(hb + result_rows_off(n, F));
    a.probe_src = (const unsigned char *)ctx->probe_src;
    a.probe_dst = (unsigned char *)ctx->probe_dst;
    a.probe_stride_a = ctx->probe_stride_a, a.probe_off_b = ctx->probe_off_b, a.probe_stride_b = ctx->probe_stride_b;
  }
  const bool gated = ctx->gate_stage_taken && projected && ctx->gate_stage.stack == a.stack && ctx->gate_stage.lds == a.lds &&
                     ctx->gate_stage.accepted == a.accepted && ctx->gate_stage.stack_accepted_only == a.stack_accepted_only;
  if (ctx->gate_stage_taken && !gated) {
    set_last_error("plv_msckf_update_resident: the batch was gated inside its Jacobian launch for other buffers than this update's");
    return PLV_E_BADARG;
  }
  if (gated) {
    ctx->skip_word = ctx->skip_word ? ctx->gate_stage.n_acc : nullptr;
    plv_ctx_update_state::AccWords &aw = us->acc_of(fdim);
    us->acc_word_used = aw.word;
    aw.z_ptr = resbuf.p, aw.z_n = n, aw.z_word = 3 - aw.word;
  } else {
    us->acc_word_used = 1;
    TRY(launch_chi2(ctx, F, a, mp_max));
  }
  us->last_route = 0;
  us->redo_w.armed = false;
  if (probe) {
    if (ctx->probe_hook) ctx->probe_hook(ctx->probe_hook_arg);
    TRY(sync(ctx));
    const unsigned char *hacc = (const unsigned char *)(hpin.as<char>() + (size_t)n * 8 + 16);
    int any = 0;
    for (int f = 0; f < F; ++f) any |= hacc[f];
    if (!any) {
      memset(hpin.p, 0, (size_t)n * 8 + 16);
      ctx->probe_done = true;
      return aux_join();
    }
    const int *hrows = (const int *)(hpin.as<char>() + result_rows_off(n, F));
    int m_acc = 0;
    for (int f = 0; f < F; ++f) m_acc += std::max(hrows[f], 0);
    if (whiten && m_acc > 0 && m_acc <= k && ekf_fast_fits(m_acc) && !plv::knob(plv::PLV_KNOB_FORCE_FACTOR_FORM)) {
      TRY(ctx->d_stackc.reserve((size_t)m_acc * nc * 8));
      TRY(launch_stack_compact(ctx, ctx->stack_of(fdim).as<double>(), Mtot, nc, d_acc_rows, F, mp_max, ctx->d_stackc.as<double>(), m_acc, true));
      TRY(aux_join());
      const double *Hc = ctx->d_stackc.as<double>();
      TRY(launch_ekf_fast(ctx, ctx->d_P.as<double>(), n, n, Hc, m_acc, k, m_acc, us->bcols_of(fdim).as<int>(), Hc + (size_t)k * m_acc, nullptr, d_dx, d_flag,
                          gathers_valid, resbuf.p, hpin.p, (rb + 3) & ~(size_t)3));
      us->last_route = 0;
      return PLV_OK;
    }
    if (whiten && !prefetched) TRY(start_prior());
  }

  const double *dH, *dr;
  int r, ldh;
  if (whiten) {
    TRY(launch_gram_information(ctx, ctx->stack_of(fdim).as<double>(), Mtot, nc, d_acc_rows, F, mp_max));
    TRY(aux_join());
    TRY(launch_ekf_whitened(ctx, ctx->d_P.as<double>(), n, n, k, us->bcols_of(fdim).as<int>(), d_dx, d_flag, resbuf.p, hpin.p, (rb + 3) & ~(size_t)3));
    us->last_route = 4;
    us->redo_w = plv_ctx_update_state::RedoW{!us->graph_mode, Mtot, k, n, F, mp_max, fdim, tmp_elems, rb, d_dx, d_flag, d_acc_rows};
    return PLV_OK;
  }
  if (Mtot > k) {
    double *R;
    int ldr;
    if (projected && d_acc_rows && !plv::knob(plv::PLV_KNOB_TSQR_TREE)) {
      TRY(ctx->d_stackc.reserve((size_t)Mtot * nc * 8));
      TRY(ctx->d_count_words.reserve(64));
      int *m_dev = ctx->d_count_words.as<int>();
      TRY(launch_stack_compact(ctx, ctx->stack_of(fdim).as<double>(), Mtot, nc, d_acc_rows, F, mp_max, ctx->d_stackc.as<double>(), Mtot, false, m_dev));
      TRY(launch_tsqr(ctx, ctx->d_stackc.as<double>(), Mtot, Mtot, nc, ctx->d_stack2.as<double>(), tmp_elems, &R, &ldr, m_dev));
    } else {
      TRY(launch_tsqr(ctx, ctx->stack_of(fdim).as<double>(), Mtot, Mtot, nc, ctx->d_stack2.as<double>(), tmp_elems, &R, &ldr));
    }
    dH = R;
    dr = R + (size_t)k * ldr;
    r = k;
    ldh = ldr;
    us->last_route = 2;
  } else {
    dH = ctx->stack_of(fdim).as<double>();
    dr = dH + (size_t)k * Mtot;
    r = Mtot;
    ldh = Mtot;
  }
  if (ekf_fast_fits(r)) {
    TRY(launch_ekf_fast(ctx, ctx->d_P.as<double>(), n, n, dH, r, k, ldh, us->bcols_of(fdim).as<int>(), dr, nullptr, d_dx, d_flag, true,
                        resbuf.p, hpin.p, (rb + 3) & ~(size_t)3));
    return PLV_OK;
  }
  TRY(launch_ekf(ctx, ctx->d_P.as<double>(), n, n, dH, r, k, ldh, us->bcols_of(fdim).as<int>(), dr, nullptr, d_dx, d_flag, true));
  TRY(d2h(ctx, hpin.p, resbuf.p, rb));
    return PLV_OK;
  };
  if (us->graph_mode && !ctx->prof.on) {
    plv_ctx_update_state::GraphKey key{ctx->d_P.p, wHf, us->brows.p, us->bcols_of(fdim).p, resbuf.p, hpin.p, ctx->mirror2_src, ctx->mirror2_dst,
                                       (const void *)(d_flag + 1), ctx->mirror2_bytes, F, fdim + 16 * (projected ? 1 : 0) + 32 * (gathers_valid ? 1 : 0), k, ld, n, mp_max,
                                       sigma2, chi2_mult, res_norm_gate, plv::alloc_epoch().load()};
    if (us->gexec && key == us->gkey) {
      PLV_HIP_CHECK(hipGraphLaunch(us->gexec, ctx->stream));
      ++us->graph_replays;
    } else if (us->gseen && key == us->gkey_seen) {
      if (us->gexec) {
        (void)hipGraphExecDestroy(us->gexec);
        us->gexec = nullptr;
      }
      hipGraph_t g = nullptr;
      PLV_HIP_CHECK(hipStreamBeginCapture(ctx->stream, hipStreamCaptureModeRelaxed));
      const int crc = enqueue();
      const hipError_t ce = hipStreamEndCapture(ctx->stream, &g);
      if (crc != PLV_OK || ce != hipSuccess || !g || plv::alloc_epoch().load() != key.epoch) {
        if (g) (void)hipGraphDestroy(g);
        us->gseen = false;
        if (crc != PLV_OK) return crc;
        TRY(enqueue());
      } else {
        const hipError_t ie = hipGraphInstantiate(&us->gexec, g, nullptr, nullptr, 0);
        (void)hipGraphDestroy(g);
        if (ie != hipSuccess) {
          us->gexec = nullptr;
          us->gseen = false;
          TRY(enqueue());
        } else {
          us->gkey = key;
          ++us->graph_captures;
          PLV_HIP_CHECK(hipGraphLaunch(us->gexec, ctx->stream));
        }
      }
    } else {
      TRY(enqueue());
      us->gkey_seen = key;
      us->gkey_seen.epoch = plv::alloc_epoch().load();
      us->gseen = true;
    }
  } else {
    const int erc = enqueue();
    const int jrc = aux_join();
    if (erc) return erc;
    if (jrc) return jrc;
  }
  ctx->gate_stage.on = 0, ctx->gate_stage_taken = false;
  ++ctx->gather_stamp;
  us->pending_fdim = fdim;
  us->pending_F = F;
  if (!us->done_ev) PLV_HIP_CHECK(hipEventCreateWithFlags(&us->done_ev, hipEventDisableTiming));
  PLV_HIP_CHECK(hipEventRecord(us->done_ev, ctx->stream));
  us->done_stamp = ctx->gather_stamp;
  return PLV_OK;
}

int plv_update_compression_mode(plv_ctx *ctx, int mode, int *last_route, int *last_ambiguous) {
  REQUIRE_CTX(ctx);
  auto *us = ustate(ctx);
  if (mode >= 0) {
    if (mode > 1) return PLV_E_BADARG;
    us->compress_mode = mode;
  }
  if (last_route) *last_route = us->last_route;
  if (last_ambiguous) *last_ambiguous = us->last_ambiguous;
  return us->compress_mode;
}

int plv_update_graph_mode(plv_ctx *ctx, int on, int *captures, int *replays) {
  REQUIRE_CTX(ctx);
  auto *us = ustate(ctx);
  if (on >= 0) {
    us->graph_mode = on != 0;
    if (!us->graph_mode && us->gexec) {
      (void)hipGraphExecDestroy(us->gexec);
      us->gexec = nullptr;
      us->gseen = false;
    }
  }
  if (captures) *captures = us->graph_captures;
  if (replays) *replays = us->graph_replays;
  return PLV_OK;
}

int plv_msckf_update_resident_wait(plv_ctx *ctx, uint8_t *accepted, int *n_accepted_rows, double *dx) {
  REQUIRE_CTX(ctx);
  auto *us = ustate(ctx);
  const int F = us->pending_F, n = ctx->cov_n, wfdim = us->pending_fdim;
  plv::PinBuf &hpin = ctx->res_pin(us->pending_fdim);
  if (F < 1 || !dx) {
    set_last_error("plv_msckf_update_resident_wait: nothing was launched");
    return PLV_E_BADARG;
  }
  us->pending_F = 0;
  if (ctx->probe_done)
    ctx->probe_done = false;
  else if (ctx->prof.on || !us->done_ev)
    TRY(sync(ctx));
  else
// ... 82 lines not shown
```

### pl-viwo_amd/csrc/plv_ctx.hpp

```cpp
#pragma once
#include <hip/hip_runtime.h>
#include <sys/resource.h>

#include "gate_stage.hpp"
#include <cstdint>
#include <cstdio>
#include <execinfo.h>
#include <cstring>
#include <algorithm>
#include <atomic>
#include <chrono>
#include <cstdlib>
#include <mutex>
#include <string>
#include <unordered_map>
#include <vector>

#include "../../include/plviwo.h"

namespace plv {

void set_last_error(const char *fmt, ...);

#define PLV_HIP_CHECK(expr)                                                              \
  do {                                                                                   \
    hipError_t _e = (expr);                                                              \
    if (_e != hipSuccess) {                                                              \
      plv::set_last_error("%s:%d %s -> %s", __FILE__, __LINE__, #expr, hipGetErrorString(_e)); \
      return PLV_E_DEVICE;                                                               \
    }                                                                                    \
  } while (0)

struct Counters {
  std::atomic<unsigned long long> launches{0}, syncs{0}, copies{0}, copy_bytes{0}, lk_iters{0}, lines_detected{0};
  std::atomic<unsigned long long> frame_ns{0}, sync_ns{0};
  std::atomic<unsigned long long> flow_wait_ns{0}, points_ns{0}, points_wait_ns{0}, lines_ns{0}, line_join_ns{0};
  std::atomic<unsigned long long> w_wake_ns{0}, w_maps_ns{0}, w_extract_ns{0}, w_feed_start_ns{0}, w_feed_ns{0};
  std::atomic<unsigned long long> chained{0};
  std::atomic<unsigned long long> spec_over[3] = {};
  std::atomic<unsigned long long> speculated{0};
  std::atomic<unsigned long long> route[8] = {};
};
inline Counters &counters() {
  static Counters c;
  return c;
}
inline int spec_grid(int max_sel) { return 2 * (max_sel > 0 ? max_sel : 1); }
inline hipError_t stream_sync(hipStream_t s) {
  ++counters().syncs;
  return hipStreamSynchronize(s);
}
inline hipError_t event_sync(hipEvent_t e) {
  ++counters().syncs;
  return hipEventSynchronize(e);
}
inline hipError_t memcpy_async(void *dst, const void *src, size_t bytes, hipMemcpyKind kind, hipStream_t s) {
  ++counters().copies;
  counters().copy_bytes += bytes;
  return hipMemcpyAsync(dst, src, bytes, kind, s);
}

enum : unsigned { PLV_KNOB_PRIOR_LATE = 2u, PLV_KNOB_GATE_SEPARATE = 1024u, PLV_KNOB_NO_CHAIN = 2048u, PLV_KNOB_CHAIN_ALWAYS = 4096u,
                  PLV_KNOB_FORCE_FACTOR_FORM = 8192u,
                  PLV_KNOB_HOST_TIMING = 1u << 14,
                  PLV_KNOB_LINE_TIMING = 1u << 15,
                  PLV_KNOB_UPDATE_TIMING = 1u << 16,
                  PLV_KNOB_KERNEL_STAMPS = 1u << 17,
                  PLV_KNOB_CHAIN_EVENTS = 1u << 18,
                  PLV_KNOB_ALLOC_DEBUG = 1u << 19,
                  PLV_KNOB_HOST_FAULTS = 1u << 20,
                  PLV_KNOB_NO_SPECULATION = 1u << 24,
                  PLV_KNOB_HELPER_NAPS = 1u << 28,
                  PLV_KNOB_TSQR_TREE = 1u << 29 };
inline std::atomic<unsigned> &knobs() {
  static std::atomic<unsigned> k{getenv("PLV_DEBUG_KNOBS") ? (unsigned)strtoul(getenv("PLV_DEBUG_KNOBS"), nullptr, 0) : 0u};
  return k;
}
inline bool knob(unsigned bit) { return (knobs().load(std::memory_order_relaxed) & bit) != 0; }
inline bool alloc_debug() { return knob(PLV_KNOB_ALLOC_DEBUG); }

struct HostPhases {
  struct Rec {
    const char *label;
    double us = 0;
    long n = 0;
    float last[64] = {};
    void put(double v) {
      last[n & 63] = (float)v;
      us += v;
      ++n;
    }
    double median() const {
      float tmp[64];
      const int m = (int)(n < 64 ? n : 64);
      for (int i = 0; i < m; ++i) tmp[i] = last[i];
      std::sort(tmp, tmp + m);
      return m ? tmp[m / 2] : 0.0;
    }
  };
  bool on = knob(PLV_KNOB_HOST_TIMING);
  std::mutex mtx;
  std::vector<Rec> recs;
  void add(const char *label, double us) {
    std::lock_guard<std::mutex> lk(mtx);
    for (auto &r : recs)
      if (r.label == label) {
        r.put(us);
        return;
      }
    for (auto &r : recs)
      if (!strcmp(r.label, label)) {
        r.put(us);
        return;
      }
    recs.push_back(Rec{label});
    recs.back().put(us);
  }
  ~HostPhases() {
    if (!on) return;
    for (auto &r : recs)
      fprintf(stderr, "[plv host] %-44s %8ld calls  %9.1f us/call  (median of the last %d: %.1f)\n", r.label, r.n, r.us / (double)r.n, (int)(r.n < 64 ? r.n : 64), r.median());
  }
};
inline HostPhases &host_phases() {
  static HostPhases h;
  return h;
}
inline std::atomic<long long> &frame_t0_ns() {
  static std::atomic<long long> t{0};
  return t;
}
inline void frame_mark(const char *label) {
  if (!host_phases().on) return;
  const long long now = std::chrono::duration_cast<std::chrono::nanoseconds>(std::chrono::steady_clock::now().time_since_epoch()).count();
  const long long t0 = frame_t0_ns().load(std::memory_order_relaxed);
  if (t0) host_phases().add(label, (double)(now - t0) * 1e-3);
}
struct NsScope {
  std::atomic<unsigned long long> &acc;
  std::chrono::steady_clock::time_point t0 = std::chrono::steady_clock::now();
  explicit NsScope(std::atomic<unsigned long long> &a) : acc(a) {}
  ~NsScope() { acc += (unsigned long long)std::chrono::duration_cast<std::chrono::nanoseconds>(std::chrono::steady_clock::now() - t0).count(); }
};
inline long thread_minor_faults() {
  struct rusage ru;
  getrusage(RUSAGE_THREAD, &ru);
  return ru.ru_minflt;
}
struct HostPhase {
  const char *label;
  std::chrono::steady_clock::time_point t0;
  long f0 = 0;
  bool on;
  static bool faults() {
    return knob(PLV_KNOB_HOST_FAULTS);
  }
  explicit HostPhase(const char *l) : label(l), on(l && host_phases().on) {
    if (on && faults()) f0 = thread_minor_faults();
    if (on) t0 = std::chrono::steady_clock::now();
  }
  void stop() {
    if (!on) return;
    if (faults())
      host_phases().add(label, (double)(thread_minor_faults() - f0));
    else
      host_phases().add(label, std::chrono::duration<double, std::micro>(std::chrono::steady_clock::now() - t0).count());
    on = false;
  }
  ~HostPhase() { stop(); }
};

struct Roctx {
  int (*push)(const char *) = nullptr;
  int (*pop)() = nullptr;
  Roctx();
};
inline Roctx &roctx() {
  static Roctx r;
  return r;
}
struct RoctxRange {
  bool on;
  explicit RoctxRange(const char *label) : on(roctx().push != nullptr) {
    if (on) roctx().push(label);
  }
  void stop() {
    if (on) roctx().pop();
    on = false;
  }
  ~RoctxRange() { stop(); }
};

inline std::atomic<unsigned long long> &alloc_epoch() {
  static std::atomic<unsigned long long> e{0};
  return e;
}

struct MemoryBook {
  std::atomic<long long> dev{0}, pin{0}, dev_peak{0}, pin_peak{0};
  std::atomic<int> growth_percent{200}, dev_floor_kb{1024}, pin_floor_kb{256};
  void add(std::atomic<long long> &now, std::atomic<long long> &peak, long long bytes) {
    const long long v = now.fetch_add(bytes) + bytes;
    long long p = peak.load();
    while (v > p && !peak.compare_exchange_weak(p, v)) {
    }
  }
  size_t sized(size_t bytes, int floor_kb) const {
    const size_t grown = (size_t)((double)bytes * std::max(100, growth_percent.load()) / 100.0) + 256;
    return std::max(grown, (size_t)std::max(0, floor_kb) << 10);
  }
};
inline MemoryBook &memory_book() {
  static MemoryBook b;
  return b;
}

struct DevBuf {
  void *p = nullptr;
  size_t cap = 0;
  int reserve(size_t bytes) {
    if (bytes <= cap) return PLV_OK;
    ++alloc_epoch();
    if (alloc_debug()) {
      fprintf(stderr, "[plv alloc] device buffer %p: %zu -> %zu bytes asked\n", (void *)this, cap, bytes);
      void *bt[8];
      backtrace_symbols_fd(bt, backtrace(bt, 8), 2);
// ... 243 lines not shown
```

### pl-viwo_amd/csrc/update_kernels.hip

```cpp
#include <algorithm>

#include "plv_ctx.hpp"
#include "blocked_chol.hpp"
#include "mfma_tile.hpp"
#include "nullspace_core.hpp"
#include "update_kernels.hpp"

namespace plv {

template <class FA, class FB>
__device__ __forceinline__ d4 mfma_tile_f64(FA a, FB b, int K, d4 acc) {
  const int lane = threadIdx.x & 63;
  const int ij = lane & 15, kq = lane >> 4;
  int k0 = 0;
  for (; k0 + 16 <= K; k0 += 16) {
    double av[4], bv[4];
#pragma unroll
    for (int u = 0; u < 4; ++u) {
      av[u] = a(ij, k0 + 4 * u + kq);
      bv[u] = b(k0 + 4 * u + kq, ij);
    }
#pragma unroll
    for (int u = 0; u < 4; ++u) acc = __builtin_amdgcn_mfma_f64_16x16x4f64(av[u], bv[u], acc, 0, 0, 0);
  }
// ... 434 lines not shown
      for (int e = t; e < 1024; e += HQ_T) {
        double x = 0.0;
#pragma unroll
        for (int w = 0; w < 8; ++w) x += buf[(w * 4 + (e >> 8)) * 256 + (e & 255)];
        Wm[e >> 8][(e >> 4) & 15][e & 15] = x;
      }
      __syncthreads();
      for (int e = t; e < 1024; e += HQ_T) {
        const int g = e >> 8, i = (e >> 4) & 15, jj = e & 15;
        double x = 0.0;
        for (int l = 0; l <= i; ++l) x += Tm[l][i] * Wm[g][l][jj];
        W2[g][i][jj] = x;
      }
      __syncthreads();
      for (int rb = wave; rb * 16 < mp; rb += 8) {
        const int r0 = d0 + rb * 16;
        const int ri = min(rb * 16 + (lane & 15), mp - 1);
        double av[4], old[4][4];
#pragma unroll
        for (int u = 0; u < 4; ++u) av[u] = Vg[(size_t)(4 * u + (lane >> 4)) * ldv + ri];
#pragma unroll
        for (int g = 0; g < 4; ++g)
#pragma unroll
          for (int q = 0; q < 4; ++q) {
            const int row = min(r0 + (lane >> 4) + 4 * q, m - 1), col = min(tc0 + 16 * g + (lane & 15), nc - 1);
            old[g][q] = A[(size_t)col * lda + row];
          }
#pragma unroll
        for (int g = 0; g < 4; ++g)
          if (g < ng) {
            d4 acc = {0, 0, 0, 0};
#pragma unroll
            for (int u = 0; u < 4; ++u) acc = __builtin_amdgcn_mfma_f64_16x16x4f64(av[u], W2[g][4 * u + (lane >> 4)][lane & 15], acc, 0, 0, 0);
#pragma unroll
            for (int q = 0; q < 4; ++q) {
              const int row = r0 + (lane >> 4) + 4 * q, col = tc0 + 16 * g + (lane & 15);
              if (row < m && col < nc) A[(size_t)col * lda + row] = old[g][q] - acc[q];
            }
          }
      }
      __syncthreads();
    }
  }
  __syncthreads();
  for (int i = t; i < nc; i += HQ_T) sg[i] = (sign_fix && A[(size_t)i * lda + i] < 0.0) ? -1.0 : 1.0;
  __syncthreads();
  for (int idx = t; idx < nc * nc; idx += HQ_T) {
    const int j = idx / nc, i = idx - j * nc;
    double *e = A + (size_t)j * lda + i;
    const double x = i > j ? 0.0 : (sg[i] < 0.0 ? -*e : *e);
    if (Rout)
      Rout[(size_t)j * ldro + (size_t)blockIdx.x * nc + i] = x;
    else
      *e = x;
  }
}

__global__ void __launch_bounds__(256) gather_cov_kernel(GatherArgs g) { gather_cov_block(g, blockIdx.x); }

__global__ void __launch_bounds__(256) chi2_t_kernel(Chi2Args a, int mt_max) {
  if (a.n_acc && blockIdx.x == 0 && threadIdx.x == 0) {
    a.n_acc[0] = 0;
    a.n_acc[2] = 0;
  }
  const int kt = (a.k + 15) >> 4;
  const int wid = blockIdx.x * 4 + (threadIdx.x >> 6);
  const int per_f = mt_max * kt;
  const int f = wid / per_f;
  if (f >= a.F) return;
  const int t = wid - f * per_f, ti = t / kt, tj = t - ti * kt;
  const int mp = a.rows[f] - a.fdim_off;
  if (ti * 16 >= mp) return;
  const int k = a.k, ld = a.ld;
  const double *H = a.Hx + (size_t)f * k * ld;
  double *T = a.T + (size_t)f * k * ld;
  const int lane = threadIdx.x & 63;
  d4 acc = {0, 0, 0, 0};
  const double *Hr = H + min(ti * 16 + (lane & 15), mp - 1);
  const double *Pq = a.Ps + min(tj * 16 + (lane & 15), k - 1);
  auto fa = [&](int, int kk) { return Hr[kk * ld]; };
  auto fb = [&](int kk, int) { return Pq[(size_t)kk * k]; };
  acc = mfma_tile_f64_pipe<16>(fa, fb, k, acc);
#pragma unroll
  for (int q = 0; q < 4; ++q) {
    const int i = ti * 16 + (lane >> 4) + 4 * q, j = tj * 16 + (lane & 15);
    if (i < mp && j < k) T[(size_t)j * ld + i] = acc[q];
  }
}

__global__ void __launch_bounds__(256) ekf_mt_kernel(const double *__restrict__ H, int ldh, int r, int k,
                                                     const int *__restrict__ cols, const double *__restrict__ P,
                                                     int ldp, int n, double *__restrict__ Mt, int ldm,
                                                     int *__restrict__ flag, const int *__restrict__ skip) {
  if (flag && blockIdx.x == 0 && threadIdx.x == 0) {
    flag[0] = 0;
  }
  if (skip && *skip == 0) return;
  const int tr_n = (r + 15) >> 4, tn_n = (n + 15) >> 4;
  const int tile = blockIdx.x * 4 + (threadIdx.x >> 6);
  if (tile >= tr_n * tn_n) return;
  const int tr = tile / tn_n, tn = tile - tr * tn_n;
  const int lane = threadIdx.x & 63;
  d4 acc = {0, 0, 0, 0};
  const double *Hr = H + min(tr * 16 + (lane & 15), r - 1);
  const double *Pq = P + min(tn * 16 + (lane & 15), n - 1);
  auto fa = [&](int, int kk) { return Hr[(size_t)kk * ldh]; };
  auto fb = [&](int kk, int) { return Pq[(size_t)kk * ldp]; };
  acc = mfma_tile_f64_pipe<16>(fa, fb, k, acc);
#pragma unroll
  for (int q = 0; q < 4; ++q) {
    int i = tr * 16 + (lane >> 4) + 4 * q, j = tn * 16 + (lane & 15);
    if (i < r && j < n) {
      Mt[(size_t)j * ldm + i] = acc[q];
      const int pos = cols[j];
      if (pos >= 0) Mt[(size_t)(n + 1 + pos) * ldm + i] = acc[q];
    }
  }
}

__global__ void __launch_bounds__(256) ekf_s_kernel(const double *__restrict__ Mt, int ldm, const double *__restrict__ H,
                                                    int ldh, int r, int k, const int *__restrict__ cols,
                                                    const double *__restrict__ Rdiag, double *__restrict__ S, int lds_, const int *__restrict__ skip) {
  if (skip && *skip == 0) return;
  const int tn = (r + 15) >> 4;
  const int tile = blockIdx.x * 4 + (threadIdx.x >> 6);
  if (tile >= tn * tn) return;
  const int ti = tile / tn, tj = tile - ti * tn;
  const int lane = threadIdx.x & 63;
  d4 acc = {0, 0, 0, 0};
  const double *Mr = Mt + min(ti * 16 + (lane & 15), r - 1);
  const double *Hr = H + min(tj * 16 + (lane & 15), r - 1);
  auto fa = [&](int, int kk) { return Mr[(size_t)kk * ldm]; };
  auto fb = [&](int kk, int) { return Hr[(size_t)kk * ldh]; };
  acc = mfma_tile_f64_pipe<16>(fa, fb, k, acc);
#pragma unroll
  for (int q = 0; q < 4; ++q) {
    int i = ti * 16 + (lane >> 4) + 4 * q, j = tj * 16 + (lane & 15);
    if (i < r && j < r) S[(size_t)j * lds_ + i] = acc[q] + (i == j ? (Rdiag ? Rdiag[i] : 1.0) : 0.0);
  }
}

struct WhitenPanels {
  const double *P;
  int ldp, n;
  const int *cols;
  const double *g;
  double *Y0;
  double *GP;
  double *d0;
  const int *use_m;
  int first;
};

__global__ void __launch_bounds__(512) ekf_ms_kernel(const double *__restrict__ H, int ldh, int r, int k, const double *__restrict__ Pc,
                                                     int ldp, int n, const double *__restrict__ Ps, double *__restrict__ Mt, int ldm,
                                                     const double *__restrict__ Rdiag, double *__restrict__ S, int lds_,
                                                     int mt_blocks, int *__restrict__ flag, const int *__restrict__ skip, int h_upper,
                                                     WhitenPanels wp) {
  __shared__ double strip[192 * 17];
  if (flag && blockIdx.x == 0 && threadIdx.x == 0) {
    flag[0] = 0;
  }
  if (skip && *skip == 0) return;
  const int wave = threadIdx.x >> 6, lane = threadIdx.x & 63, li = lane & 15, nw = blockDim.x >> 6;
  if ((int)blockIdx.x < mt_blocks) {
    const int tr_n = (r + 15) >> 4, tn_n = (n + 15) >> 4;
    const int tile = blockIdx.x * nw + wave;
    if (tile >= tr_n * tn_n) return;
    const int tr = tile / tn_n, tn = tile - tr * tn_n;
    d4 acc = {0, 0, 0, 0};
    const int k0 = h_upper ? min(tr * 16, k) : 0;
    const double *Hr = H + min(tr * 16 + li, r - 1) + (size_t)k0 * ldh;
    const double *Pq = Pc + min(tn * 16 + li, n - 1) + (size_t)k0 * ldp;
    auto fa = [&](int, int kk) { return Hr[(size_t)kk * ldh]; };
    auto fb = [&](int kk, int) { return Pq[(size_t)kk * ldp]; };
    acc = mfma_tile_f64_pipe<16>(fa, fb, k - k0, acc);
#pragma unroll
    for (int q = 0; q < 4; ++q) {
      const int i = tr * 16 + (lane >> 4) + 4 * q, j = tn * 16 + li;
      if (i < r && j < n) Mt[(size_t)j * ldm + i] = acc[q];
    }
    return;
  }
  const int kt = (k + 15) >> 4, tr_n = (r + 15) >> 4;
  if (wp.first >= 0 && (int)blockIdx.x >= wp.first) {
    __shared__ int scols[192];
    if ((wp.use_m[0] | wp.use_m[1]) == 0) return;
    const int b0 = ((int)blockIdx.x - wp.first) * 16, bl = min(b0 + li, wp.n - 1);
    if (threadIdx.x < 192) scols[threadIdx.x] = wp.cols[min((int)threadIdx.x, k - 1)];
    __syncthreads();
    for (int tj = wave; tj < kt; tj += nw) {
      d4 acc = {0, 0, 0, 0};
      const double *Gr = Ps + min(tj * 16 + li, k - 1);
      auto fa = [&](int, int kk) { return Gr[(size_t)kk * k]; };
      auto fb = [&](int kk, int) { return wp.P[(size_t)scols[kk] * wp.ldp + bl]; };
      acc = mfma_tile_f64_pipe<16>(fa, fb, k, acc);
#pragma unroll
      for (int q = 0; q < 4; ++q) {
        const int c = tj * 16 + (lane >> 4) + 4 * q;
        if (c < k) strip[c * 17 + li] = acc[q];
        if (c < k && b0 + li < wp.n) wp.GP[(size_t)(b0 + li) * k + c] = acc[q];
      }
    }
    if (wave == nw - 1) {
      double sum = 0.0;
      for (int c = lane >> 4; c < k; c += 4) sum += wp.P[(size_t)scols[c] * wp.ldp + bl] * wp.g[c];
      sum += __shfl_xor(sum, 16);
      sum += __shfl_xor(sum, 32);
      if (lane < 16 && b0 + li < wp.n) wp.d0[b0 + li] = sum;
    }
    __syncthreads();
    for (int tj = wave; tj < kt; tj += nw) {
      d4 acc = {0, 0, 0, 0};
      const int k0 = min(tj * 16, k);
      const double *Hr = H + min(tj * 16 + li, k - 1) + (size_t)k0 * ldh;
      const double *sp = strip + k0 * 17;
      auto fa = [&](int, int kk) { return Hr[(size_t)kk * ldh]; };
      auto fb = [&](int kk, int) { return sp[kk * 17 + li]; };
      acc = mfma_tile_f64_pipe<16>(fa, fb, k - k0, acc);
#pragma unroll
      for (int q = 0; q < 4; ++q) {
        const int c = tj * 16 + (lane >> 4) + 4 * q;
        if (c < k && b0 + li < wp.n) wp.Y0[(size_t)(b0 + li) * k + c] = acc[q];
      }
    }
    return;
  }
  const int ti = blockIdx.x - mt_blocks;
  {
    const int k0 = h_upper ? min(ti * 16, k) : 0;
    const double *Hr = H + min(ti * 16 + li, r - 1) + (size_t)k0 * ldh;
    for (int tj = wave; tj < kt; tj += nw) {
      d4 acc = {0, 0, 0, 0};
      const double *Pq = Ps + min(tj * 16 + li, k - 1) + (size_t)k0 * k;
      auto fa = [&](int, int kk) { return Hr[(size_t)kk * ldh]; };
      auto fb = [&](int kk, int) { return Pq[(size_t)kk * k]; };
      acc = mfma_tile_f64_pipe<16>(fa, fb, k - k0, acc);
#pragma unroll
      for (int q = 0; q < 4; ++q) {
        const int j = tj * 16 + li;
        if (j < k) strip[j * 17 + (lane >> 4) + 4 * q] = acc[q];
      }
    }
  }
  __syncthreads();
  for (int tj = ti + wave; tj < tr_n; tj += nw) {
    d4 acc = {0, 0, 0, 0};
    const int k0 = h_upper ? min(tj * 16, k) : 0;
    const double *Hc = H + min(tj * 16 + li, r - 1) + (size_t)k0 * ldh;
    const double *sp = strip + k0 * 17;
    auto fa = [&](int, int kk) { return sp[kk * 17 + li]; };
    auto fb = [&](int kk, int) { return Hc[(size_t)kk * ldh]; };
    acc = mfma_tile_f64_pipe<16>(fa, fb, k - k0, acc);
#pragma unroll
    for (int q = 0; q < 4; ++q) {
      const int i = ti * 16 + (lane >> 4) + 4 * q, j = tj * 16 + li;
      if (i < r && j < r) S[(size_t)j * lds_ + i] = acc[q] + (i == j ? (Rdiag ? Rdiag[i] : 1.0) : 0.0);
    }
  }
}

__global__ void __launch_bounds__(1024) ekf_chol_kernel(const double *__restrict__ S, int lds_, int r, double *__restrict__ L,
                                                        int ldl, int *__restrict__ flag) {
  extern __shared__ double smem[];
  const int rp = r | 1;
  double *A = smem;
  for (int idx = threadIdx.x; idx < r * r; idx += blockDim.x) {
    int j = idx / r, i = idx - j * r;
    if (i >= j) A[i * rp + j] = S[(size_t)i * lds_ + j];
  }
  __syncthreads();
  bool bad = false;
  for (int j = 0; j < r; ++j) {
    const double d = A[j * rp + j];
    if (!(d > 0.0)) bad = true;
    const double inv = 1.0 / d;
    const int nrem = r - 1 - j;
    for (int idx = threadIdx.x; idx < nrem * nrem; idx += blockDim.x) {
      int ci = idx / nrem, ii = idx - ci * nrem;
      int c = j + 1 + ci, i = j + 1 + ii;
      if (i >= c) A[i * rp + c] -= A[i * rp + j] * A[c * rp + j] * inv;
    }
    __syncthreads();
  }
  for (int idx = threadIdx.x; idx < r * r; idx += blockDim.x) {
    int j = idx / r, i = idx - j * r;
    double val = 0.0;
    if (i >= j) {
      double sq = sqrt(A[j * rp + j]);
      val = (i == j) ? sq : A[i * rp + j] / sq;
    }
    L[(size_t)j * ldl + i] = val;
  }
  if (bad && threadIdx.x == 0) atomicOr(flag, 2);
}

__global__ void __launch_bounds__(256) ekf_trsm_kernel(const double *__restrict__ L, int ldl, int r,
                                                       const double *__restrict__ Mt, int ldm, int n,
                                                       const double *__restrict__ res, const double *__restrict__ P,
                                                       int ldp, double *__restrict__ W, int ldw, int *__restrict__ flag) {
  extern __shared__ double smem[];
  const int rp = r | 1;
  double *Ls = smem;
  for (int idx = threadIdx.x; idx < r * r; idx += blockDim.x) {
    int p = idx / r, q = idx - p * r;
    Ls[q * rp + p] = L[(size_t)p * ldl + q];
  }
  __syncthreads();
  const int col = blockIdx.x * 4 + (threadIdx.x >> 6);
  if (col > n) return;
  const int lane = threadIdx.x & 63;
  const double *b = col < n ? Mt + (size_t)col * ldm : res;
  double x0 = 0.0, x1 = 0.0, x2 = 0.0, x3 = 0.0;
  double ssq = 0.0;
  for (int q = 0; q < r; ++q) {
    double part = 0.0;
    if (lane < q) part += Ls[q * rp + lane] * x0;
    if (lane + 64 < q) part += Ls[q * rp + lane + 64] * x1;
    if (lane + 128 < q) part += Ls[q * rp + lane + 128] * x2;
    if (lane + 192 < q) part += Ls[q * rp + lane + 192] * x3;
    const double sum = wave_sum(part);
    const double xq = (b[q] - sum) / Ls[q * rp + q];
    ssq += xq * xq;
    const int slot = q >> 6, owner = q & 63;
    if (lane == owner) {
      if (slot == 0) x0 = xq;
      else if (slot == 1) x1 = xq;
      else if (slot == 2) x2 = xq;
      else x3 = xq;
      W[(size_t)col * ldw + q] = xq;
    }
  }
  if (col < n && lane == 0) {
    if (P[(size_t)col * ldp + col] - ssq < 0.0) atomicOr(flag, 1);
  }
}

__global__ void __launch_bounds__(256) ekf_apply_kernel(const double *__restrict__ W, int ldw, int r, int n,
                                                        double *__restrict__ P, int ldp, double *__restrict__ dx,
                                                        const int *__restrict__ flag) {
  if (*flag != 0) return;
  const int tn = (n + 15) >> 4;
  const int ntri = tn * (tn + 1) / 2;
  const int wid = blockIdx.x * 4 + (threadIdx.x >> 6);
  const int lane = threadIdx.x & 63;
  if (wid < ntri) {
    int ti = 0, rem = wid;
    while (rem >= tn - ti) {
      rem -= tn - ti;
      ++ti;
    }
    const int tj = ti + rem;
    d4 acc = {0, 0, 0, 0};
    auto fa = [&](int i, int kk) { int c = ti * 16 + i; return c < n ? W[(size_t)c * ldw + kk] : 0.0; };
    auto fb = [&](int kk, int j) { int c = tj * 16 + j; return c < n ? W[(size_t)c * ldw + kk] : 0.0; };
    acc = mfma_tile_f64(fa, fb, r, acc);
#pragma unroll
    for (int q = 0; q < 4; ++q) {
      int i = ti * 16 + (lane >> 4) + 4 * q, j = tj * 16 + (lane & 15);
      if (i < n && j < n && i <= j) {
        double val = P[(size_t)j * ldp + i] - acc[q];
        P[(size_t)j * ldp + i] = val;
        P[(size_t)i * ldp + j] = val;
      }
    }
  } else {
    const int w = wid - ntri;
    const int i = w * 64 + lane;
    if (i < n) {
      const double *y = W + (size_t)n * ldw;
      double s = 0.0;
      for (int q = 0; q < r; ++q) s += W[(size_t)i * ldw + q] * y[q];
      dx[i] = s;
    }
  }
}

static inline int cdiv(int a, int b) { return (a + b - 1) / b; }

int gather_args(plv_ctx *ctx, const double *d_P, int n, int ldp, const int *d_cols, int k, GatherArgs &g) {
  int rc;
  if ((rc = ctx->d_Pc.reserve((size_t)k * n * 8)) || (rc = ctx->d_Ps.reserve((size_t)k * k * 8)) ||
      (rc = ctx->d_inv.reserve((size_t)n * 4)))
    return rc;
  g = GatherArgs{d_P, ldp, n, d_cols, k, ctx->d_Pc.as<double>(), ctx->d_Ps.as<double>(), ctx->d_inv.as<int>()};
  ++ctx->gather_stamp;
  return PLV_OK;
}

int launch_nullspace(plv_ctx *ctx, int F, int fdim, int k, int ld, const int *d_rows, double *d_Hf, double *d_Hx,
                     double *d_res, const double *d_P, int n, int ldp, const int *d_cols, int shift) {
  size_t shm = (size_t)(ld * (fdim + k + 1) + ld) * sizeof(double);
  if (shm > 160 * 1024) {
    set_last_error("nullspace: feature block of %zu bytes exceeds LDS", shm);
    return PLV_E_CAPACITY;
  }
  GatherArgs g{};
  int extra = 0;
  if (d_P) {
    int rc = gather_args(ctx, d_P, n, ldp, d_cols, k, g);
    if (rc) return rc;
    extra = cdiv(std::max(k * n, std::max(k * k, n)), 256);
  }
  PLV_HIP_CHECK(ensure_dyn_smem((const void *)nullspace_kernel, (int)shm));
  ProfScope ps(ctx->prof, "nullspace_kernel", ctx->stream);
  hipLaunchKernelGGL(nullspace_kernel, dim3(F + extra), dim3(256), shm, ctx->stream, fdim, k, ld, d_rows, d_Hf, d_Hx, d_res, F, g,
                     shift < 0 ? fdim : shift);
  PLV_HIP_CHECK(hipGetLastError());
  return PLV_OK;
}

int launch_gather_cov(plv_ctx *ctx, const double *d_P, int n, int ldp, const int *d_cols, int k) {
  GatherArgs g{};
  int rc = gather_args(ctx, d_P, n, ldp, d_cols, k, g);
  if (rc) return rc;
  ProfScope ps(ctx->prof, "gather_cov_kernel", ctx->stream);
  hipLaunchKernelGGL(gather_cov_kernel, dim3(cdiv(std::max(k * n, std::max(k * k, n)), 256)), dim3(256), 0, ctx->stream, g);
  PLV_HIP_CHECK(hipGetLastError());
  return PLV_OK;
}

int launch_chi2(plv_ctx *ctx, int F, const Chi2Args &a_in, int max_mp) {
  if (max_mp > CHI2_MAXM) {
    set_last_error("chi2: %d projected rows per feature exceeds %d", max_mp, CHI2_MAXM);
    return PLV_E_CAPACITY;
  }
  Chi2Args a = a_in;
  int rc;
  if ((rc = ctx->d_T.reserve_units((size_t)F, (size_t)std::max(ctx->cfg.num_features, 64), (size_t)a.k * a.ld * 8))) return rc;
  a.F = F;
  a.Ps = ctx->d_Ps.as<double>();
  a.T = ctx->d_T.as<double>();
  const int mt = (max_mp + 15) / 16, kt = (a.k + 15) / 16;
  {
    ProfScope ps(ctx->prof, "chi2_t_kernel", ctx->stream);
    hipLaunchKernelGGL(chi2_t_kernel, dim3(cdiv(F * mt * kt, 4)), dim3(256), 0, ctx->stream, a, mt);
  }
  size_t shm = (size_t)(65 * 65 + 8) * sizeof(double);
  ProfScope ps(ctx->prof, "chi2_gate_kernel", ctx->stream);
  if (max_mp <= 32) {
    PLV_HIP_CHECK(ensure_dyn_smem((const void *)chi2_gate_kernel<2>, (int)shm));
    hipLaunchKernelGGL(chi2_gate_kernel<2>, dim3(F), dim3(256), shm, ctx->stream, a);
  } else {
    PLV_HIP_CHECK(ensure_dyn_smem((const void *)chi2_gate_kernel<4>, (int)shm));
    hipLaunchKernelGGL(chi2_gate_kernel<4>, dim3(F), dim3(320), shm, ctx->stream, a);
  }
  PLV_HIP_CHECK(hipGetLastError());
  return PLV_OK;
}

int launch_tsqr(plv_ctx *ctx, double *d_A, int lda, int m, int nc, double *d_tmp, size_t tmp_elems, double **result,
                int *ld_out, const int *m_dev) {
  {
    const int cap = HQ_T * 4, nb = m <= HQ_T * 2 ? 1 : (m + cap - 1) / cap;
    const int ldv = ((nb == 1 ? m : cap) + 63) & ~63;
    const size_t v_elems = (size_t)nb * ldv * 16, r_elems = nb > 1 ? (size_t)nb * nc * nc : 0;
    const int ldv2 = (nb * nc + 63) & ~63;
    const size_t need = v_elems + r_elems + (nb > 1 ? (size_t)ldv2 * 16 : 0);
    const bool tree_holds = ((size_t)nc * nc + QR_CHUNK + 8) * sizeof(double) <= 160 * 1024 && nc * QR_PARTS <= 1024;
    if ((2 * m >= 3 * nc || m_dev || !tree_holds) && m >= nc && nc <= 208 && nb <= 8 && need <= tmp_elems && !(plv::knob(plv::PLV_KNOB_TSQR_TREE) && tree_holds)) {
      ProfScope ps(ctx->prof, "hqr_kernel", ctx->stream);
      double *Vg = d_tmp, *Rst = d_tmp + v_elems, *Vg2 = Rst + r_elems;
      const int ldro = nb * nc;
      if (nb == 1 && m <= HQ_T * 2)
        hipLaunchKernelGGL(hqr_kernel<2>, dim3(1), dim3(HQ_T), 0, ctx->stream, d_A, lda, m, nc, 1, Vg, ldv, m_dev, (double *)nullptr, 0, (const int *)nullptr, 0, 0);
      else
        hipLaunchKernelGGL(hqr_kernel<4>, dim3(nb), dim3(HQ_T), 0, ctx->stream, d_A, lda, m, nc, nb == 1 ? 1 : 2, Vg, ldv, m_dev, nb > 1 ? Rst : (double *)nullptr,
                           ldro, (const int *)nullptr, 0, 0);
      if (nb > 1) {
        if (ldro <= HQ_T * 2)
          hipLaunchKernelGGL(hqr_kernel<2>, dim3(1), dim3(HQ_T), 0, ctx->stream, Rst, ldro, ldro, nc, 1, Vg2, ldv2, (const int *)nullptr, (double *)nullptr, 0, m_dev, m, cap);
        else
          hipLaunchKernelGGL(hqr_kernel<4>, dim3(1), dim3(HQ_T), 0, ctx->stream, Rst, ldro, ldro, nc, 1, Vg2, ldv2, (const int *)nullptr, (double *)nullptr, 0, m_dev, m, cap);
      }
      PLV_HIP_CHECK(hipGetLastError());
      *result = nb > 1 ? Rst : d_A;
      *ld_out = nb > 1 ? ldro : lda;
      return PLV_OK;
    }
  }
  size_t shm = ((size_t)nc * nc + QR_CHUNK + 8) * sizeof(double);
  if (shm > 160 * 1024 || nc * QR_PARTS > 1024) {
    set_last_error("tsqr: %d columns exceed the LDS-resident R capacity", nc);
    return PLV_E_CAPACITY;
  }
  PLV_HIP_CHECK(ensure_dyn_smem((const void *)qr_accum_kernel, (int)shm));
  int threads = cdiv(nc * QR_PARTS, 64) * 64;
  double *src = d_A, *dst = d_tmp;
  size_t cap_src = (size_t)lda * nc, cap_dst = tmp_elems;
  int src_ld = lda, rows = m;
  int rpw = cdiv(2 * nc, QR_CHUNK) * QR_CHUNK;
  for (;;) {
    int W = cdiv(rows, rpw);
    if (W < 1) W = 1;
    int ldo = W * nc;
    if ((size_t)ldo * nc > cap_dst) {
      set_last_error("tsqr: workspace too small (%d x %d > %zu)", ldo, nc, cap_dst);
      return PLV_E_CAPACITY;
    }
    {
      ProfScope ps(ctx->prof, "qr_accum_kernel", ctx->stream);
      hipLaunchKernelGGL(qr_accum_kernel, dim3(W), dim3(threads), shm, ctx->stream, src, src_ld, rows, nc, rpw, dst, ldo,
                         W == 1 ? 1 : 0);
    }
    PLV_HIP_CHECK(hipGetLastError());
    if (W == 1) {
      *result = dst;
      *ld_out = ldo;
      return PLV_OK;
    }
    rows = W * nc;
    src_ld = ldo;
    double *t = src;
    src = dst;
    dst = t;
    size_t tc = cap_src;
    cap_src = cap_dst;
    cap_dst = tc;
  }
}

void launch_ekf_ms(plv_ctx *ctx, const double *d_P, int n, int ldp, const double *d_H, int r, int k, int ldh,
                   const int *d_cols, const double *d_Rdiag, double *Mt, int ldm, double *S, bool gathered, int *d_flag) {
  if (!gathered) (void)launch_gather_cov(ctx, d_P, n, ldp, d_cols, k);
  ProfScope ps(ctx->prof, "ekf_ms_kernel", ctx->stream);
  const int mt_blocks = cdiv(cdiv(r, 16) * cdiv(n, 16), 4);
  if (k > 192) {
    hipLaunchKernelGGL(ekf_mt_kernel, dim3(mt_blocks), dim3(256), 0, ctx->stream, d_H, ldh, r, k, ctx->d_inv.as<int>(),
                       ctx->d_Pc.as<double>(), n, n, Mt, ldm, d_flag, ctx->skip_word);
    hipLaunchKernelGGL(ekf_s_kernel, dim3(cdiv(cdiv(r, 16) * cdiv(r, 16), 4)), dim3(256), 0, ctx->stream, Mt + (size_t)(n + 1) * ldm, ldm,
                       d_H, ldh, r, k, d_cols, d_Rdiag, S, r, ctx->skip_word);
    return;
  }
  hipLaunchKernelGGL(ekf_ms_kernel, dim3(mt_blocks + cdiv(r, 16)), dim3(256), 0, ctx->stream, d_H, ldh, r, k, ctx->d_Pc.as<double>(), n, n,
                     ctx->d_Ps.as<double>(), Mt, ldm, d_Rdiag, S, r, mt_blocks, d_flag, ctx->skip_word, 0, WhitenPanels{nullptr, 0, 0, nullptr, nullptr, nullptr, nullptr, nullptr, nullptr, -1});
}

void launch_whiten_b(plv_ctx *ctx, const double *Lt, int k, const double *Gs, const double *gv, double *cv, double *B, int *d_flag,
                     const double *d_P, int ldp, int n, const int *d_cols, double *Y0, double *GP, double *d0, const int *use_m) {
  ProfScope ps(ctx->prof, "ekf_ms_kernel", ctx->stream);
  const int mt_blocks = cdiv(cdiv(k, 16), 8), first = mt_blocks + cdiv(k, 16);
  hipLaunchKernelGGL(ekf_ms_kernel, dim3(first + cdiv(n, 16)), dim3(512), 0, ctx->stream, Lt, k, k, k, gv, 1, 1, Gs, cv, k,
                     (const double *)nullptr, B, k, mt_blocks, d_flag, ctx->skip_word, 1, WhitenPanels{d_P, ldp, n, d_cols, gv, Y0, GP, d0, use_m, first});
}

int launch_ekf(plv_ctx *ctx, double *d_P, int n, int ldp, const double *d_H, int r, int k, int ldh, const int *d_cols,
               const double *d_res, const double *d_Rdiag, double *d_dx, int *d_flag, bool gathered) {
  int rc;
  const int ldm = r, ldw = r;
  if ((rc = ctx->d_Mt.reserve((size_t)r * (n + 1 + k) * 8)) || (rc = ctx->d_S.reserve((size_t)r * r * 8 * 2)) ||
      (rc = ctx->d_W.reserve((size_t)r * (n + 1) * 8)))
    return rc;
  double *Mt = ctx->d_Mt.as<double>(), *S = ctx->d_S.as<double>(), *L = S + (size_t)r * r, *W = ctx->d_W.as<double>();
  size_t shm = (size_t)r * (r | 1) * sizeof(double);
  if (shm > 160 * 1024) {
    set_last_error("ekf: r=%d exceeds the LDS-resident Cholesky capacity", r);
    return PLV_E_CAPACITY;
  }
  launch_ekf_ms(ctx, d_P, n, ldp, d_H, r, k, ldh, d_cols, d_Rdiag, Mt, ldm, S, gathered, d_flag);
  PLV_HIP_CHECK(ensure_dyn_smem((const void *)ekf_chol_kernel, (int)shm));
  PLV_HIP_CHECK(ensure_dyn_smem((const void *)ekf_trsm_kernel, (int)shm));
  {
    ProfScope ps(ctx->prof, "ekf_chol_kernel", ctx->stream);
    hipLaunchKernelGGL(ekf_chol_kernel, dim3(1), dim3(1024), shm, ctx->stream, S, r, r, L, r, d_flag);
  }
  {
    ProfScope ps(ctx->prof, "ekf_trsm_kernel", ctx->stream);
    hipLaunchKernelGGL(ekf_trsm_kernel, dim3(cdiv(n + 1, 4)), dim3(256), shm, ctx->stream, L, r, r, Mt, ldm, n, d_res, d_P,
                       ldp, W, ldw, d_flag);
  }
  {
    ProfScope ps(ctx->prof, "ekf_apply_kernel", ctx->stream);
    int tn = cdiv(n, 16);
    int waves = tn * (tn + 1) / 2 + cdiv(n, 64);
    hipLaunchKernelGGL(ekf_apply_kernel, dim3(cdiv(waves, 4)), dim3(256), 0, ctx->stream, W, ldw, r, n, d_P, ldp, d_dx,
                       d_flag);
  }
  PLV_HIP_CHECK(hipGetLastError());
  return PLV_OK;
}

}
```

### pl-viwo_amd/csrc/update_kernels.hpp

```cpp
#pragma once
#include "plv_ctx.hpp"

namespace plv {

struct Chi2Args {
  const double *P;
  int ldp;
  int k, ld, fdim_off;
  const int *rows;
  const double *Hx, *res;
  const int *cols;
  double sigma2;
  double *chi2;
  double *dec;
  double *stack;
  int lds, mp_max;
  double chi2_mult, res_norm_gate;
  const double *q95;
  int q95_n;
  int min_rows;
  unsigned char *accepted;
  int *acc_rows;
  int *n_acc;
  int stack_accepted_only;
  int F;
  const double *Ps;
  double *T;
  unsigned char *h_accepted;
  int *h_acc_rows;
  const unsigned char *probe_src;
  unsigned char *probe_dst;
  int probe_stride_a, probe_off_b, probe_stride_b;
};

int launch_nullspace(plv_ctx *ctx, int F, int fdim, int k, int ld, const int *d_rows, double *d_Hf, double *d_Hx,
                     double *d_res, const double *d_P = nullptr, int n = 0, int ldp = 0, const int *d_cols = nullptr,
                     int shift = -1 );
struct GatherArgs;
int gather_args(plv_ctx *ctx, const double *d_P, int n, int ldp, const int *d_cols, int k, GatherArgs &g);
int launch_gather_cov(plv_ctx *ctx, const double *d_P, int n, int ldp, const int *d_cols, int k);
int launch_chi2(plv_ctx *ctx, int F, const Chi2Args &a, int max_mp);
int launch_tsqr(plv_ctx *ctx, double *d_A, int lda, int m, int nc, double *d_tmp, size_t tmp_elems, double **result,
                int *ld_out, const int *m_dev = nullptr);
int launch_ekf(plv_ctx *ctx, double *d_P, int n, int ldp, const double *d_H, int r, int k, int ldh, const int *d_cols,
               const double *d_res, const double *d_Rdiag, double *d_dx, int *d_flag, bool gathered = false);

void launch_ekf_ms(plv_ctx *ctx, const double *d_P, int n, int ldp, const double *d_H, int r, int k, int ldh,
                   const int *d_cols, const double *d_Rdiag, double *Mt, int ldm, double *S, bool gathered = false,
                   int *d_flag = nullptr);
bool ekf_fast_fits(int r);
int launch_ekf_fast(plv_ctx *ctx, double *d_P, int n, int ldp, const double *d_H, int r, int k, int ldh, const int *d_cols,
                    const double *d_res, const double *d_Rdiag, double *d_dx, int *d_flag, bool gathered = false, const void *mirror_src = nullptr,
                    void *mirror_dst = nullptr, size_t mirror_bytes = 0);

void launch_whiten_b(plv_ctx *ctx, const double *Lt, int k, const double *Gs, const double *gv, double *cv, double *B, int *d_flag,
                     const double *d_P, int ldp, int n, const int *d_cols, double *Y0, double *GP, double *d0, const int *use_m);
int launch_stack_compact(plv_ctx *ctx, const double *d_A, int lda, int nc, const int *d_acc_rows, int F, int mp_max, double *d_dst, int ldd, bool exact_rows = false,
                         int *d_total_out = nullptr );
int launch_cov_restore(plv_ctx *ctx, double *d_P, int n, const double *save, const unsigned *save_word, unsigned seq);
int launch_stack_zero_rejected(plv_ctx *ctx, double *d_A, int lda, int nc, const int *d_acc_rows, int F, int mp_max);
int launch_prior_factor(plv_ctx *ctx, hipStream_t st, const double *d_P, int n, int ldp, const int *d_cols, int k);
int launch_gram_information(plv_ctx *ctx, const double *d_A, int lda, int nc, const int *d_acc_rows, int F, int mp_max);
int launch_ekf_whitened(plv_ctx *ctx, double *d_P, int n, int ldp, int k, const int *d_cols, double *d_dx, int *d_flag, const void *mirror_src, void *mirror_dst,
                        size_t mirror_bytes);
int launch_bchol_prior(plv_ctx *ctx, hipStream_t st, const double *d_P, int ldp, int n, const int *d_cols, int k, double *d_Lt, int ldl,
                       double *d_W0, int ldw, int *d_n_near);

struct WhitenC1Args {
  const double *P;
  int ldp;
  const int *cols;
  const double *GP;
  double *C1;
  const double *Y0;
  const int *use_m;
};
int launch_bchol_ekf(plv_ctx *ctx, const double *d_S, int lds_, int r, const double *d_Mt, int ldm, int n,
                     const double *d_res, double *d_W, int ldw, int *d_flag, const WhitenC1Args *wc = nullptr);

}
```

Measured before the change: 2153.

## Widen fused Jacobian kernels to 512 threads and read EKF rows through a segment map

The fused point and line Jacobian/nullspace kernels launch with 512 threads instead of 256. Their strided loops and the gate tail now scale with blockDim, while pose-row writes and the gather blocks stay limited to the original waves. Separately, the whitened EKF path passes a small segment table of accepted feature rows into the EKF measurement kernel so it reads the stacked matrix in place. This skips the stack-compaction launch, and the residual column is copied into Mt. Calibration loads become wave-uniform via readfirstlane. The risks are register pressure at 512 threads and per-row map lookup overhead.

Result: slower. 1883 (-12.6%).

```diff
diff --git a/pl-viwo_amd/csrc/dense_kernels.hip b/pl-viwo_amd/csrc/dense_kernels.hip
--- a/pl-viwo_amd/csrc/dense_kernels.hip
+++ b/pl-viwo_amd/csrc/dense_kernels.hip
@@ -140,14 +140,16 @@
 
 int launch_ekf_fast(plv_ctx *ctx, double *d_P, int n, int ldp, const double *d_H, int r, int k, int ldh, const int *d_cols,
                     const double *d_res, const double *d_Rdiag, double *d_dx, int *d_flag, bool gathered, const void *mirror_src,
-                    void *mirror_dst, size_t mirror_bytes) {
+                    void *mirror_dst, size_t mirror_bytes, const EkfRowMap *map) {
   int rc;
   const int ldm = r, ldw = r;
+  if (map && (!map->n || k > 192)) return PLV_E_BADARG;
   if ((rc = ctx->d_Mt.reserve((size_t)r * (n + 1 + k) * 8)) || (rc = ctx->d_S.reserve((size_t)r * r * 8 * 2)) ||
       (rc = ctx->d_W.reserve((size_t)r * (n + 1) * 8)) || (rc = ctx->d_y.reserve((size_t)n * n * 8)))
     return rc;
   double *Mt = ctx->d_Mt.as<double>(), *S = ctx->d_S.as<double>(), *W = ctx->d_W.as<double>(), *dC = ctx->d_y.as<double>();
-  launch_ekf_ms(ctx, d_P, n, ldp, d_H, r, k, ldh, d_cols, d_Rdiag, Mt, ldm, S, gathered, d_flag);
+  launch_ekf_ms(ctx, d_P, n, ldp, d_H, r, k, ldh, d_cols, d_Rdiag, Mt, ldm, S, gathered, d_flag, map);
+  if (map) d_res = Mt + (size_t)n * ldm;
   if ((rc = launch_bchol_ekf(ctx, S, r, r, Mt, ldm, n, d_res, W, ldw, d_flag))) return rc;
   {
     ProfScope ps(ctx->prof, "ekf_dc_kernel", ctx->stream);
diff --git a/pl-viwo_amd/csrc/gate_core.hpp b/pl-viwo_amd/csrc/gate_core.hpp
--- a/pl-viwo_amd/csrc/gate_core.hpp
+++ b/pl-viwo_amd/csrc/gate_core.hpp
@@ -75,7 +75,7 @@
 
 __device__ __forceinline__ void gate_tail(const GateStage &g, GateLds &L, const double *Ps, double *T, int f, const double *X, int ncol, int fdim,
                                           int shift, int rows, int k, const int *cols_g) {
-  const int wave = threadIdx.x >> 6, lane = threadIdx.x & 63, li = lane & 15, lq = lane >> 4;
+  const int wave = threadIdx.x >> 6, nwaves = blockDim.x >> 6, lane = threadIdx.x & 63, li = lane & 15, lq = lane >> 4;
   const int mp = rows - fdim;
   const bool valid = shift == fdim && mp >= 1 && mp <= GATE_MMAX && rows >= g.min_rows;
   if (f == 0 && threadIdx.x == 0 && g.n_acc_next) *g.n_acc_next = 0;
@@ -90,7 +90,7 @@
     }
     const int mt = (mp + 15) >> 4, kt = (k + 15) >> 4;
     const int ngroups = (k + 15) >> 4;
-    for (int tj = wave; tj < kt; tj += 4) {
+    for (int tj = wave; tj < kt; tj += nwaves) {
       const int jb = min(tj * 16 + li, k - 1);
       double bv[GATE_KMAX / 4];
 #pragma unroll
@@ -120,7 +120,7 @@
     }
     __syncthreads();
     GATE_STAMP(6);
-    for (int t = wave; t < mt * mt; t += 4) {
+    for (int t = wave; t < mt * mt; t += nwaves) {
       const int ti = t / mt, tj = t - ti * mt;
       if (tj < ti) continue;
       const double *Tr = T + (size_t)min(ti * 16 + li, mp - 1) * GATE_TLD;
@@ -178,7 +178,7 @@
     double *dst = g.stack + (size_t)f * g.mp_max;
     const int rows_w = g.stack_accepted_only ? mp : g.mp_max;
     for (int i = threadIdx.x & 31; i < rows_w; i += 32)
-      for (int j = threadIdx.x >> 5; j <= k; j += 8) {
+      for (int j = threadIdx.x >> 5; j <= k; j += blockDim.x >> 5) {
         double v = 0.0;
         if (pass && i < mp) v = Hp[(size_t)i * ncol + j];
         dst[(size_t)j * g.lds + i] = v;
diff --git a/pl-viwo_amd/csrc/jacobian_kernels.hip b/pl-viwo_amd/csrc/jacobian_kernels.hip
--- a/pl-viwo_amd/csrc/jacobian_kernels.hip
+++ b/pl-viwo_amd/csrc/jacobian_kernels.hip
@@ -791,7 +791,7 @@
       double WI[12];
 #pragma unroll
       for (int q = 0; q < 12; ++q) WI[q] = pr[PRE_WI + q];
-      rows_write_pose(P.clone_col[s0_l[i] + wave], c, WI, ldM(pr + PRE_HO + 9 * wave), pr[PRE_LAM + wave], hx, 1, ncol);
+      if (wave < 4) rows_write_pose(P.clone_col[s0_l[i] + wave], c, WI, ldM(pr + PRE_HO + 9 * wave), pr[PRE_LAM + wave], hx, 1, ncol);
       if (wave == 0) {
         double Wm[4], r2[2] = {pr[PRE_R2], pr[PRE_R2 + 1]}, dtj[6];
 #pragma unroll
@@ -812,7 +812,7 @@
 #pragma unroll
         for (int q = 0; q < 16; ++q) dzeta[q] = pr[PRE_DZETA + q];
         rows_write_int(P, c, Wm, dzeta, hx, 1, ncol);
-      } else {
+      } else if (wave == 3) {
         double wz[6];
 #pragma unroll
         for (int q = 0; q < 6; ++q) wz[q] = pr[PRE_WZ + q];
@@ -840,14 +840,14 @@
 }
 static_assert(sizeof(WinTab) % 8 == 0, "fused_lds_layout counts WinTab in doubles");
 
-__global__ void __launch_bounds__(256) __attribute__((amdgpu_waves_per_eu(2))) jacobian_nullspace_kernel(JacParams P, int F, GatherArgs g, PointTriStage tri, GateStage gate) {
+__global__ void __launch_bounds__(512) __attribute__((amdgpu_waves_per_eu(2))) jacobian_nullspace_kernel(JacParams P, int F, GatherArgs g, PointTriStage tri, GateStage gate) {
   extern __shared__ double jsm[];
   __shared__ int s_rows, s_base;
   __shared__ double tri_tot[32], s_tri[5];
   __shared__ double s_ct[JAC_MAX_WIN / 2 + 3];
   __shared__ int s_ccol[JAC_MAX_WIN / 2 + 3];
   if ((int)blockIdx.x >= F) {
-    gather_cov_block(g, blockIdx.x - F);
+    if (threadIdx.x < 256) gather_cov_block(g, blockIdx.x - F);
     return;
   }
   int f = blockIdx.x;
@@ -857,7 +857,7 @@
   }
   const int wave = threadIdx.x >> 6, lane = threadIdx.x & 63;
   double touch = 0.0;
-  for (int off = threadIdx.x * 128; off < P.in_bytes; off += 256 * 128) touch += *(const volatile double *)(P.in_base + off);
+  for (int off = threadIdx.x * 128; off < P.in_bytes; off += blockDim.x * 128) touch += *(const volatile double *)(P.in_base + off);
   const int ld = P.ld, k = P.k, ncol = 3 + k + 1, max_obs = tri.max_obs;
   const FusedLds lay = fused_lds_layout(ld, ncol, 3, 2 * max(P.n_clones - 3, 0), max_obs, tri.on != 0);
   double *X = jsm, *piv = jsm + lay.ns, *tri_smem = jsm + lay.tri, *pre = jsm + lay.pre, *cam = jsm + lay.cam;
@@ -915,7 +915,7 @@
       triangulate_feature(P, f, 0, o1 - o0, cam, valid_l, uvn_l, uv_l, tri.opt, tri.p_out, tri.ok_out, tri.err_out, max_obs, tri_smem, tri_tot, true, s_tri);
     }
   } else {
-    for (int i = threadIdx.x - 64; i < o1 - o0; i += 192) {
+    for (int i = threadIdx.x - 64; i < o1 - o0; i += blockDim.x - 64) {
       const int c = slot_l[i];
       if (c < 0) continue;
       Interp jac;
@@ -923,7 +923,7 @@
       interpolate_tab(P, tab[2 * s0 + 1], s0, tm_l[i] + P.cam_dt, true, jac);
       pre_store_jac(pre + (size_t)c * PRE_STRIDE, jac);
     }
-    if (gate.on) gate_stage_prior(gate, reinterpret_cast<double *>(reinterpret_cast<char *>(jsm) + gate.ps_off), P.cols_in, k, threadIdx.x - 64, 192);
+    if (gate.on) gate_stage_prior(gate, reinterpret_cast<double *>(reinterpret_cast<char *>(jsm) + gate.ps_off), P.cols_in, k, threadIdx.x - 64, blockDim.x - 64);
   }
   __threadfence_block();
   __syncthreads();
@@ -1642,7 +1642,7 @@
     const int o = o0 + i;
     double *pr = pre + (size_t)max(c, 0) * LPRE_STRIDE;
     M3 A00, A30, A03;
-    M3 Re, Rsk;
+    M3 &Re = A00, &Rsk = A30;
     if (c >= 0) {
       if (wave == 0) {
         line_fej_part(nG, vG, ldM(pr + PRE_R), ldV(pr + PRE_P), A00, A30, A03);
@@ -1673,7 +1673,7 @@
       double WI[12];
 #pragma unroll
       for (int q = 0; q < 12; ++q) WI[q] = pr[LPRE_WI + q];
-      rows_write_pose(P.clone_col[s0_l[i] + wave], c, WI, ldM(pr + PRE_HO + 9 * wave), pr[PRE_LAM + wave], hx, 1, ncol);
+      if (wave < 4) rows_write_pose(P.clone_col[s0_l[i] + wave], c, WI, ldM(pr + PRE_HO + 9 * wave), pr[PRE_LAM + wave], hx, 1, ncol);
       if (wave == 0) {
         double Wm[4], r2[2] = {pr[LPRE_R2], pr[LPRE_R2 + 1]}, dtj[6];
 #pragma unroll
@@ -1691,6 +1691,11 @@
     }
     __syncthreads();
   }
+}
+
+__device__ __forceinline__ double wave_uniform_f64(double v) {
+  const int lo = __builtin_amdgcn_readfirstlane(__double2loint(v)), hi = __builtin_amdgcn_readfirstlane(__double2hiint(v));
+  return __hiloint2double(hi, lo);
 }
 
 __device__ __forceinline__ void jpl_left_update_dev(const double *Qin, const double *d, double *M) {
@@ -1717,7 +1722,7 @@
   M[6] = 2 * w * y + 2 * z * x, M[7] = -2 * w * x + 2 * z * y, M[8] = c + 2 * z * z;
 }
 
-__global__ void __launch_bounds__(256) line_jacobian_nullspace_kernel(JacParams P, int L, GatherArgs g, JacParams Pt, LineTriStage tri, GateStage gate) {
+__global__ void __launch_bounds__(512) line_jacobian_nullspace_kernel(JacParams P, int L, GatherArgs g, JacParams Pt, LineTriStage tri, GateStage gate) {
   extern __shared__ double jsm[];
   __shared__ int s_rows, s_base, s_ok;
   __shared__ double s_line[6];
@@ -1727,12 +1732,12 @@
   __shared__ unsigned char s_has;
   if (P.chain_dx && *P.chain_status != 0) return;
   if ((int)blockIdx.x >= L) {
-    gather_cov_block(g, blockIdx.x - L);
+    if (threadIdx.x < 256) gather_cov_block(g, blockIdx.x - L);
     return;
   }
   const int l = blockIdx.x, wave = threadIdx.x >> 6, lane = threadIdx.x & 63;
   double touch = 0.0;
-  for (int off = threadIdx.x * 128; off < P.in_bytes; off += 256 * 128) touch += *(const volatile double *)(P.in_base + off);
+  for (int off = threadIdx.x * 128; off < P.in_bytes; off += blockDim.x * 128) touch += *(const volatile double *)(P.in_base + off);
   const int ld = P.ld, k = P.k, ncol = 6 + k + 1, max_obs = tri.max_obs, nwin = max(P.n_clones - 3, 0);
   const FusedLds lay = fused_lds_layout(ld, ncol, 6, (tri.on ? 3 : 2) * nwin, max_obs, tri.on != 0);
   double *X = jsm, *piv = jsm + lay.ns, *pre = jsm + lay.pre, *cam = jsm + lay.cam, *imu = cam + (size_t)max_obs * 12;
@@ -1793,12 +1798,12 @@
     __syncthreads();
     P.clone_R = s_cR, P.clone_p = s_cp;
 #pragma unroll
-    for (int q = 0; q < 9; ++q) P.R_ItoC[q] = s_cal[q];
-#pragma unroll
-    for (int q = 0; q < 3; ++q) P.p_IinC[q] = s_cal[9 + q];
-#pragma unroll
-    for (int q = 0; q < 8; ++q) P.K[q] = s_cal[12 + q];
-    P.cam_dt = s_cal[20];
+    for (int q = 0; q < 9; ++q) P.R_ItoC[q] = wave_uniform_f64(s_cal[q]);
+#pragma unroll
+    for (int q = 0; q < 3; ++q) P.p_IinC[q] = wave_uniform_f64(s_cal[9 + q]);
+#pragma unroll
+    for (int q = 0; q < 8; ++q) P.K[q] = wave_uniform_f64(s_cal[12 + q]);
+    P.cam_dt = wave_uniform_f64(s_cal[20]);
   }
   if (wave == 0) {
     const int base = assign_row_slots(P, o0, o1, ld, tm_l, s0_l, slot_l);
@@ -1857,7 +1862,7 @@
       }
     }
   } else {
-    for (int i = threadIdx.x - 64; i < o1 - o0; i += 192) {
+    for (int i = threadIdx.x - 64; i < o1 - o0; i += blockDim.x - 64) {
       const int c = slot_l[i];
       if (c < 0) continue;
       const int s0 = s0_l[i];
@@ -1873,7 +1878,7 @@
 #pragma unroll
       for (int q = 0; q < 3; ++q) pr[PRE_PE + q] = pe[q];
     }
-    if (gate.on) gate_stage_prior(gate, reinterpret_cast<double *>(reinterpret_cast<char *>(jsm) + gate.ps_off), P.cols_in, k, threadIdx.x - 64, 192);
+    if (gate.on) gate_stage_prior(gate, reinterpret_cast<double *>(reinterpret_cast<char *>(jsm) + gate.ps_off), P.cols_in, k, threadIdx.x - 64, blockDim.x - 64);
   }
   __threadfence_block();
   __syncthreads();
@@ -2082,6 +2087,8 @@
   return h;
 }
 
+static int fused_launch_width() { return knob(PLV_KNOB_FUSED_NARROW) ? 256 : 512; }
+
 int launch_line_jacobians(plv_ctx *ctx, const JacParams &P) {
   ProfScope ps(ctx->prof, "line_jacobian_kernel", ctx->stream);
   hipLaunchKernelGGL(line_jacobian_kernel, dim3(P.n_feat), dim3(64), 0, ctx->stream, P);
@@ -2120,7 +2127,7 @@
   ctx->gate_stage_taken = gate.on != 0;
   PLV_HIP_CHECK(ensure_dyn_smem((const void *)line_jacobian_nullspace_kernel, (int)shm));
   if (jac_stamps().on) TRY_STAMP(jac_stamps().arm(ctx->stream, P.n_feat));
-  hipLaunchKernelGGL(line_jacobian_nullspace_kernel, dim3(P.n_feat + (g ? gather_blocks : 0)), dim3(256), shm, ctx->stream, P, P.n_feat,
+  hipLaunchKernelGGL(line_jacobian_nullspace_kernel, dim3(P.n_feat + (g ? gather_blocks : 0)), dim3(fused_launch_width()), shm, ctx->stream, P, P.n_feat,
                      g ? *g : none, Pt ? *Pt : P, tri, gate);
   PLV_HIP_CHECK(hipGetLastError());
   if (jac_stamps().on) TRY_STAMP(jac_stamps().collect(ctx->stream, P.n_feat, 1));
@@ -2188,7 +2195,7 @@
   PLV_HIP_CHECK(ensure_dyn_smem((const void *)jacobian_nullspace_kernel, (int)shm));
   if (jac_stamps().on) TRY_STAMP(jac_stamps().arm(ctx->stream, P.n_feat));
   const int wg_feat = P.spec_order ? std::max(1, std::min(P.n_feat, spec_grid(P.max_sel))) : P.n_feat;
-  hipLaunchKernelGGL(jacobian_nullspace_kernel, dim3(wg_feat + (g ? gather_blocks : 0)), dim3(256), shm, ctx->stream, P, wg_feat,
+  hipLaunchKernelGGL(jacobian_nullspace_kernel, dim3(wg_feat + (g ? gather_blocks : 0)), dim3(fused_launch_width()), shm, ctx->stream, P, wg_feat,
                      g ? *g : none, tri, gate);
   PLV_HIP_CHECK(hipGetLastError());
   if (jac_stamps().on) TRY_STAMP(jac_stamps().collect(ctx->stream, P.n_feat, 0));
diff --git a/pl-viwo_amd/csrc/plv_api.hip b/pl-viwo_amd/csrc/plv_api.hip
--- a/pl-viwo_amd/csrc/plv_api.hip
+++ b/pl-viwo_amd/csrc/plv_api.hip
@@ -901,9 +901,23 @@
       return aux_join();
     }
     const int *hrows = (const int *)(hpin.as<char>() + result_rows_off(n, F));
-    int m_acc = 0;
-    for (int f = 0; f < F; ++f) m_acc += std::max(hrows[f], 0);
+    int m_acc = 0, n_ent = 0;
+    plv::EkfRowMap map{};
+    for (int f = 0; f < F; ++f) {
+      if (hrows[f] <= 0) continue;
+      m_acc += hrows[f];
+      if (n_ent < PLV_EKF_ROWMAP_MAX) map.base[n_ent] = f * mp_max, map.end[n_ent] = m_acc;
+      ++n_ent;
+    }
     if (whiten && m_acc > 0 && m_acc <= k && ekf_fast_fits(m_acc) && !plv::knob(plv::PLV_KNOB_FORCE_FACTOR_FORM)) {
+      if (n_ent <= PLV_EKF_ROWMAP_MAX && k <= 192 && !plv::knob(plv::PLV_KNOB_FUSED_NARROW)) {
+        map.n = n_ent;
+        TRY(aux_join());
+        TRY(launch_ekf_fast(ctx, ctx->d_P.as<double>(), n, n, ctx->stack_of(fdim).as<double>(), m_acc, k, Mtot, us->bcols_of(fdim).as<int>(), nullptr, nullptr, d_dx,
+                            d_flag, gathers_valid, resbuf.p, hpin.p, (rb + 3) & ~(size_t)3, &map));
+        us->last_route = 0;
+        return PLV_OK;
+      }
       TRY(ctx->d_stackc.reserve((size_t)m_acc * nc * 8));
       TRY(launch_stack_compact(ctx, ctx->stack_of(fdim).as<double>(), Mtot, nc, d_acc_rows, F, mp_max, ctx->d_stackc.as<double>(), m_acc, true));
       TRY(aux_join());
diff --git a/pl-viwo_amd/csrc/plv_ctx.hpp b/pl-viwo_amd/csrc/plv_ctx.hpp
--- a/pl-viwo_amd/csrc/plv_ctx.hpp
+++ b/pl-viwo_amd/csrc/plv_ctx.hpp
@@ -71,7 +71,8 @@
                   PLV_KNOB_HOST_FAULTS = 1u << 20,
                   PLV_KNOB_NO_SPECULATION = 1u << 24,
                   PLV_KNOB_HELPER_NAPS = 1u << 28,
-                  PLV_KNOB_TSQR_TREE = 1u << 29 };
+                  PLV_KNOB_TSQR_TREE = 1u << 29,
+                  PLV_KNOB_FUSED_NARROW = 1u << 30 };
 inline std::atomic<unsigned> &knobs() {
   static std::atomic<unsigned> k{getenv("PLV_DEBUG_KNOBS") ? (unsigned)strtoul(getenv("PLV_DEBUG_KNOBS"), nullptr, 0) : 0u};
   return k;
diff --git a/pl-viwo_amd/csrc/update_kernels.hip b/pl-viwo_amd/csrc/update_kernels.hip
--- a/pl-viwo_amd/csrc/update_kernels.hip
+++ b/pl-viwo_amd/csrc/update_kernels.hip
@@ -610,11 +610,19 @@
   int first;
 };
 
+__device__ __forceinline__ int ekf_map_row(const EkfRowMap &m, int i) {
+  int row = m.n ? m.base[0] + i : i;
+#pragma unroll
+  for (int e = 1; e < PLV_EKF_ROWMAP_MAX; ++e)
+    if (e < m.n && i >= m.end[e - 1]) row = m.base[e] + (i - m.end[e - 1]);
+  return row;
+}
+
 __global__ void __launch_bounds__(512) ekf_ms_kernel(const double *__restrict__ H, int ldh, int r, int k, const double *__restrict__ Pc,
                                                      int ldp, int n, const double *__restrict__ Ps, double *__restrict__ Mt, int ldm,
                                                      const double *__restrict__ Rdiag, double *__restrict__ S, int lds_,
                                                      int mt_blocks, int *__restrict__ flag, const int *__restrict__ skip, int h_upper,
-                                                     WhitenPanels wp) {
+                                                     WhitenPanels wp, EkfRowMap map) {
   __shared__ double strip[192 * 17];
   if (flag && blockIdx.x == 0 && threadIdx.x == 0) {
     flag[0] = 0;
@@ -628,7 +636,7 @@
     const int tr = tile / tn_n, tn = tile - tr * tn_n;
     d4 acc = {0, 0, 0, 0};
     const int k0 = h_upper ? min(tr * 16, k) : 0;
-    const double *Hr = H + min(tr * 16 + li, r - 1) + (size_t)k0 * ldh;
+    const double *Hr = H + ekf_map_row(map, min(tr * 16 + li, r - 1)) + (size_t)k0 * ldh;
     const double *Pq = Pc + min(tn * 16 + li, n - 1) + (size_t)k0 * ldp;
     auto fa = [&](int, int kk) { return Hr[(size_t)kk * ldh]; };
     auto fb = [&](int kk, int) { return Pq[(size_t)kk * ldp]; };
@@ -687,7 +695,9 @@
   const int ti = blockIdx.x - mt_blocks;
   {
     const int k0 = h_upper ? min(ti * 16, k) : 0;
-    const double *Hr = H + min(ti * 16 + li, r - 1) + (size_t)k0 * ldh;
+    const double *Hr = H + ekf_map_row(map, min(ti * 16 + li, r - 1)) + (size_t)k0 * ldh;
+    if (map.n && threadIdx.x < 16 && ti * 16 + (int)threadIdx.x < r)
+      Mt[(size_t)n * ldm + ti * 16 + threadIdx.x] = H[ekf_map_row(map, ti * 16 + threadIdx.x) + (size_t)k * ldh];
     for (int tj = wave; tj < kt; tj += nw) {
       d4 acc = {0, 0, 0, 0};
       const double *Pq = Ps + min(tj * 16 + li, k - 1) + (size_t)k0 * k;
@@ -705,7 +715,7 @@
   for (int tj = ti + wave; tj < tr_n; tj += nw) {
     d4 acc = {0, 0, 0, 0};
     const int k0 = h_upper ? min(tj * 16, k) : 0;
-    const double *Hc = H + min(tj * 16 + li, r - 1) + (size_t)k0 * ldh;
+    const double *Hc = H + ekf_map_row(map, min(tj * 16 + li, r - 1)) + (size_t)k0 * ldh;
     const double *sp = strip + k0 * 17;
     auto fa = [&](int, int kk) { return sp[kk * 17 + li]; };
     auto fb = [&](int kk, int) { return Hc[(size_t)kk * ldh]; };
@@ -979,7 +989,7 @@
 }
 
 void launch_ekf_ms(plv_ctx *ctx, const double *d_P, int n, int ldp, const double *d_H, int r, int k, int ldh,
-                   const int *d_cols, const double *d_Rdiag, double *Mt, int ldm, double *S, bool gathered, int *d_flag) {
+                   const int *d_cols, const double *d_Rdiag, double *Mt, int ldm, double *S, bool gathered, int *d_flag, const EkfRowMap *map) {
   if (!gathered) (void)launch_gather_cov(ctx, d_P, n, ldp, d_cols, k);
   ProfScope ps(ctx->prof, "ekf_ms_kernel", ctx->stream);
   const int mt_blocks = cdiv(cdiv(r, 16) * cdiv(n, 16), 4);
@@ -991,7 +1001,8 @@
     return;
   }
   hipLaunchKernelGGL(ekf_ms_kernel, dim3(mt_blocks + cdiv(r, 16)), dim3(256), 0, ctx->stream, d_H, ldh, r, k, ctx->d_Pc.as<double>(), n, n,
-                     ctx->d_Ps.as<double>(), Mt, ldm, d_Rdiag, S, r, mt_blocks, d_flag, ctx->skip_word, 0, WhitenPanels{nullptr, 0, 0, nullptr, nullptr, nullptr, nullptr, nullptr, nullptr, -1});
+                     ctx->d_Ps.as<double>(), Mt, ldm, d_Rdiag, S, r, mt_blocks, d_flag, ctx->skip_word, 0, WhitenPanels{nullptr, 0, 0, nullptr, nullptr, nullptr, nullptr, nullptr, nullptr, -1},
+                     map ? *map : EkfRowMap{});
 }
 
 void launch_whiten_b(plv_ctx *ctx, const double *Lt, int k, const double *Gs, const double *gv, double *cv, double *B, int *d_flag,
@@ -999,7 +1010,7 @@
   ProfScope ps(ctx->prof, "ekf_ms_kernel", ctx->stream);
   const int mt_blocks = cdiv(cdiv(k, 16), 8), first = mt_blocks + cdiv(k, 16);
   hipLaunchKernelGGL(ekf_ms_kernel, dim3(first + cdiv(n, 16)), dim3(512), 0, ctx->stream, Lt, k, k, k, gv, 1, 1, Gs, cv, k,
-                     (const double *)nullptr, B, k, mt_blocks, d_flag, ctx->skip_word, 1, WhitenPanels{d_P, ldp, n, d_cols, gv, Y0, GP, d0, use_m, first});
+                     (const double *)nullptr, B, k, mt_blocks, d_flag, ctx->skip_word, 1, WhitenPanels{d_P, ldp, n, d_cols, gv, Y0, GP, d0, use_m, first}, EkfRowMap{});
 }
 
 int launch_ekf(plv_ctx *ctx, double *d_P, int n, int ldp, const double *d_H, int r, int k, int ldh, const int *d_cols,
diff --git a/pl-viwo_amd/csrc/update_kernels.hpp b/pl-viwo_amd/csrc/update_kernels.hpp
--- a/pl-viwo_amd/csrc/update_kernels.hpp
+++ b/pl-viwo_amd/csrc/update_kernels.hpp
@@ -45,13 +45,18 @@
 int launch_ekf(plv_ctx *ctx, double *d_P, int n, int ldp, const double *d_H, int r, int k, int ldh, const int *d_cols,
                const double *d_res, const double *d_Rdiag, double *d_dx, int *d_flag, bool gathered = false);
 
+#define PLV_EKF_ROWMAP_MAX 8
+struct EkfRowMap {
+  int n;
+  int base[PLV_EKF_ROWMAP_MAX], end[PLV_EKF_ROWMAP_MAX];
+};
 void launch_ekf_ms(plv_ctx *ctx, const double *d_P, int n, int ldp, const double *d_H, int r, int k, int ldh,
                    const int *d_cols, const double *d_Rdiag, double *Mt, int ldm, double *S, bool gathered = false,
-                   int *d_flag = nullptr);
+                   int *d_flag = nullptr, const EkfRowMap *map = nullptr);
 bool ekf_fast_fits(int r);
 int launch_ekf_fast(plv_ctx *ctx, double *d_P, int n, int ldp, const double *d_H, int r, int k, int ldh, const int *d_cols,
                     const double *d_res, const double *d_Rdiag, double *d_dx, int *d_flag, bool gathered = false, const void *mirror_src = nullptr,
-                    void *mirror_dst = nullptr, size_t mirror_bytes = 0);
+                    void *mirror_dst = nullptr, size_t mirror_bytes = 0, const EkfRowMap *map = nullptr );
 
 void launch_whiten_b(plv_ctx *ctx, const double *Lt, int k, const double *Gs, const double *gv, double *cv, double *B, int *d_flag,
                      const double *d_P, int ldp, int n, const int *d_cols, double *Y0, double *GP, double *d0, const int *use_m);
```
